# Sewer56/dxt-lossless-transform

Measured on AMD Instinct MI355X. Metric: GiB/s BC blocks transformed (fwd+inv), higher is better.
Workload: dtype u8

## Files before the change

### dxt-lossless-transform_amd/csrc/batch_api.cpp

```cpp
#include <hip/hip_runtime_api.h>

#include <algorithm>
#include <condition_variable>
#include <cstdlib>
#include <cstring>
#include <exception>
#include <mutex>
#include <thread>
#include <vector>

#include "../../include/dxtlt_gfx950.h"
#include "bcn_launch.h"
#include "granule_launch.h"
#include "host_common.h"
#include "table_ring.h"

namespace {

using namespace dxtlt_host;
using dxtlt::BatchEntry;

inline uint32_t item_block_bytes(uint8_t format)
{
    return is_pixel_format(format) ? (uint32_t)pixel_bytes_of(format) : format == 1 || format == 4 ? 8u : 16u;
}

const char* const kDeviceFormatText = "batch item: format must be 1..5 (BC1..BC5), 6 (BC6H) or 7 (BC7; 6 and 7 are this build's own formats; "
                                      "pixel formats 8 and 9 go through dxtlt_transform_batch_host or the calls of dxtlt_pixels.h)";
const char* const kHostFormatText = "batch item: format must be 1..5 (BC1..BC5), 6 (BC6H), 7 (BC7), 8 (4-byte pixels) or 9 (3-byte pixels; "
                                    "6 to 9 are this build's own formats)";

inline bool pixel_item_overlaps(const DxtltBatchItem& it)
{
    if (!is_pixel_format(it.format) || it.len == 0)
        return false;
    const uintptr_t a = reinterpret_cast<uintptr_t>(it.d_input), b = reinterpret_cast<uintptr_t>(it.d_output);
    return a < b + it.len && b < a + it.len;
}

int32_t launch_pixel_item(const DxtltBatchItem& it, void* stream)
{
    const uint64_t pixels = it.len / item_block_bytes(it.format);
    return pixel_device_range(pixel_bytes_of(it.format), it.inverse != 0, it.d_input, it.d_output, pixels, 0, pixels,
                              pixel_decorrelate_of(it.decorrelation_mode),
                              pixel_layout_of(it.split_alpha_endpoints != 0, it.split_colour_endpoints != 0), stream);
}

thread_local dxtlt_host::TableRing g_ring;

const bool kTableByCopyEngine = dxtlt::experiment_env("DXTLT_BATCH_TABLE_COPY") != nullptr && dxtlt::experiment_env("DXTLT_BATCH_TABLE_COPY")[0] == '1';

}

dxtlt_host::TableRing& dxtlt_host::thread_table_ring() { return g_ring; }

hipError_t dxtlt_host::upload_table(TableSlot* slot, size_t bytes, hipStream_t stream)
{
    if (kTableByCopyEngine)
        return hipMemcpyAsync(slot->dev, slot->host, bytes, hipMemcpyHostToDevice, stream);
    return dxtlt::launch_table_upload(slot->host_mapped, slot->dev, bytes, stream);
}

namespace {

int32_t batch_device(const DxtltBatchItem* items, size_t count, void* hip_stream, bool pixels_allowed)
{
    if (count == 0)
        return kOk;
    if (items == nullptr)
        return fail(kInvalidArgument, "NULL item array with count > 0");
    for (size_t i = 0; i < count; ++i) {
        const DxtltBatchItem& it = items[i];
        if (it.format < 1 || it.format > (pixels_allowed ? 9 : 7))
            return fail(kInvalidArgument, kDeviceFormatText);
        if (it.len % item_block_bytes(it.format) != 0)
            return fail(kInvalidLength, "batch item: len is not a multiple of the block size");
        if (it.decorrelation_mode > 3 && dxtlt::format_has_colour(it.format))
            return fail(kInvalidArgument, "batch item: decorrelation_mode must be 0..3");
        if (it.len > 0 && (it.d_input == nullptr || it.d_output == nullptr))
            return fail(kInvalidArgument, "batch item: NULL device buffer with len > 0");
        if (pixel_item_overlaps(it))
            return fail(kInvalidArgument, "batch item: pixel input and output overlap");
    }
    for (const int format : {7, 6}) {
        uint64_t granules[2] = {0, 0};
        for (size_t i = 0; i < count; ++i)
            if (items[i].format == format)
                granules[items[i].inverse ? 1 : 0] += items[i].len / 16 / 1024;
        if (granules[0] > 0xFFFFFFull || granules[1] > 0xFFFFFFull)
            return fail(kInvalidArgument, dxtlt::granule::named(format, "batch too large for one launch (256 GiB or more of ", " in one direction)"));
    }
    hipStream_t user = static_cast<hipStream_t>(hip_stream);

    struct Group {
        std::vector<BatchEntry> entries;
        uint32_t wgs = 0;
        uint32_t uniform_wgs = 0;
        bool uniform = true;
    };
    constexpr int kGroups = 5 * 2 * 16;
    std::vector<Group> groups(kGroups);
    auto group_settings = [](int gi) {
        dxtlt::Settings s{};
        s.variant = (gi >> 2) & 3;
        s.split_alpha = ((gi >> 1) & 1) != 0;
        s.split_colour = (gi & 1) != 0;
        return s;
    };
    std::vector<size_t> singles;
    for (size_t i = 0; i < count; ++i) {
        const DxtltBatchItem& it = items[i];
        if (it.len == 0 || dxtlt::granule::is_granule_format(it.format) || is_pixel_format(it.format))
            continue;
        if (it.len >= (size_t(64) << 30))
            return fail(kInvalidArgument, "batch item of 64 GiB or more: use the single-buffer entry point");
        const bool colour = dxtlt::format_has_colour(it.format);
        const int sa = dxtlt::format_has_alpha_split(it.format) && it.split_alpha_endpoints ? 1 : 0;
        const int sc = colour && it.split_colour_endpoints ? 1 : 0, mode = colour ? it.decorrelation_mode : 0;
        const int gi = (((it.format - 1) * 2 + (it.inverse ? 1 : 0)) << 4) | (mode << 2) | (sa << 1) | sc;
        Group& g = groups[gi];
        BatchEntry e{};
        e.src = static_cast<const uint8_t*>(it.d_input);
        e.dst = static_cast<uint8_t*>(it.d_output);
        e.blocks = it.len / item_block_bytes(it.format);
        e.first_wg = g.wgs;
        const uint32_t wgs = dxtlt::plan_batch_entry((dxtlt::Format)it.format, it.inverse != 0, group_settings(gi), e);
        if (wgs == 0xFFFFFFFFu) {
            singles.push_back(i);
            continue;
        }
        if ((uint64_t)g.wgs + wgs > 0xFFFFFFull)
            return fail(kInvalidArgument, "batch too large for one launch (64 GiB or more of one format, direction and settings)");
        g.wgs += wgs;
        g.entries.push_back(e);
        if (g.entries.size() == 1)
            g.uniform_wgs = wgs;
        else if (wgs != g.uniform_wgs)
            g.uniform = false;
    }
    static const bool no_uniform = dxtlt::experiment_env("DXTLT_BATCH_NO_UNIFORM") != nullptr;
    static const bool no_strided = dxtlt::experiment_env("DXTLT_BATCH_NO_STRIDED") != nullptr;

    using GranuleEntry = dxtlt::granule::BatchEntry;
    struct GranulePlan {
        std::vector<GranuleEntry> entries, tails;
        std::vector<uint32_t> coarse;
        uint64_t wgs = 0;
        size_t at = 0, entry_bytes = 0, tail_bytes = 0, bytes = 0;
    };
    GranulePlan granule_plans[4];
    size_t table_bytes = 0;
    for (int q = 0; q < 4; ++q) {
        GranulePlan& p = granule_plans[q];
        const int inverse = q & 1, format = q < 2 ? 7 : 6;
        for (size_t i = 0; i < count; ++i) {
            const DxtltBatchItem& it = items[i];
            if (it.format != format || it.len == 0 || (it.inverse != 0) != (inverse != 0))
                continue;
            const uint64_t blocks = it.len / 16, tail = blocks % 1024, main = blocks - tail;
            const uint8_t* src = static_cast<const uint8_t*>(it.d_input);
            uint8_t* dst = static_cast<uint8_t*>(it.d_output);
            if (main != 0) {
                p.entries.push_back({src, dst, main, (uint32_t)p.wgs, 0});
                p.wgs += main / 1024;
            }
            if (tail != 0)
                p.tails.push_back({src + main * 16, dst + main * 16, 0, 0, (uint32_t)tail});
        }
        if (p.entries.empty() && p.tails.empty())
            continue;
        p.coarse.resize(((size_t)p.wgs + 63) / 64);
        size_t cur = 0;
        for (size_t k = 0; k < p.coarse.size(); ++k) {
            while (cur + 1 < p.entries.size() && p.entries[cur + 1].first_wg <= (uint32_t)(k * 64))
                ++cur;
            p.coarse[k] = (uint32_t)cur;
        }
        p.entry_bytes = p.entries.size() * sizeof(GranuleEntry);
        p.tail_bytes = p.tails.size() * sizeof(GranuleEntry);
        p.bytes = (p.entry_bytes + p.tail_bytes + p.coarse.size() * sizeof(uint32_t) + 15) & ~(size_t)15;
        p.at = table_bytes;
        table_bytes += p.bytes;
    }

    struct Placed {
        int gi;
        size_t at, entry_bytes;
    };
    std::vector<Placed> placed;
    for (int gi = 0; gi < kGroups; ++gi) {
        const Group& g = groups[gi];
        if (g.entries.empty())
            continue;
        const size_t entry_bytes = (g.entries.size() * sizeof(BatchEntry) + 15) & ~(size_t)15;
        placed.push_back({gi, table_bytes, entry_bytes});
        table_bytes += entry_bytes + dxtlt::batch_index_bytes(g.wgs);
    }
    if (table_bytes != 0) {
        TableSlot* slot = nullptr;
        hipError_t e = g_ring.acquire(table_bytes, &slot);
        if (e != hipSuccess)
            return fail(kDevice, "batch table staging", e);
        for (const GranulePlan& p : granule_plans) {
            if (p.bytes == 0)
                continue;
            uint8_t* h = static_cast<uint8_t*>(slot->host) + p.at;
            if (p.entry_bytes) std::memcpy(h, p.entries.data(), p.entry_bytes);
            if (p.tail_bytes) std::memcpy(h + p.entry_bytes, p.tails.data(), p.tail_bytes);
            if (!p.coarse.empty()) std::memcpy(h + p.entry_bytes + p.tail_bytes, p.coarse.data(), p.coarse.size() * sizeof(uint32_t));
        }
        std::vector<bool> wide(placed.size());
        for (size_t k = 0; k < placed.size(); ++k) {
            const Group& g = groups[placed[k].gi];
            uint8_t* h = static_cast<uint8_t*>(slot->host) + placed[k].at;
            std::memcpy(h, g.entries.data(), g.entries.size() * sizeof(BatchEntry));
            wide[k] = dxtlt::build_batch_index(g.entries.data(), g.entries.size(), g.wgs, h + placed[k].entry_bytes);
        }
        e = upload_table(slot, table_bytes, user);
        const char* what = "batch table copy / launch";
        for (int q = 0; q < 4 && e == hipSuccess; ++q) {
            const GranulePlan& p = granule_plans[q];
            const int inverse = q & 1, format = q < 2 ? 7 : 6;
            if (p.bytes == 0)
                continue;
            const uint8_t* d = static_cast<const uint8_t*>(slot->dev) + p.at;
            e = dxtlt::granule::launch_batch(format, inverse != 0, reinterpret_cast<const GranuleEntry*>(d),
                                             reinterpret_cast<const uint32_t*>(d + p.entry_bytes + p.tail_bytes), (uint32_t)p.entries.size(),
                                             (uint32_t)p.wgs, reinterpret_cast<const GranuleEntry*>(d + p.entry_bytes),
                                             (uint32_t)p.tails.size(), user);
            if (e != hipSuccess)
                what = format == 7 ? "BC7 batch table copy / launch" : "BC6H batch table copy / launch";
        }
        for (size_t k = 0; k < placed.size() && e == hipSuccess; ++k) {
            const int gi = placed[k].gi;
            Group& g = groups[gi];
            const size_t n = g.entries.size();
            const bool uniform = g.uniform && !no_uniform;
            bool strided = uniform && !no_strided;
            const int64_t src_stride = n >= 2 ? (int64_t)(g.entries[1].src - g.entries[0].src) : 0;
            const int64_t dst_stride = n >= 2 ? (int64_t)(g.entries[1].dst - g.entries[0].dst) : 0;
            for (size_t i = 1; i < n && strided; ++i) {
                const BatchEntry &a = g.entries[0], &b = g.entries[i];
                strided = b.blocks == a.blocks && b.full_tiles == a.full_tiles && b.form == a.form && b.halo_vecs == a.halo_vecs &&
                          std::memcmp(b.shift, a.shift, sizeof a.shift) == 0 && std::memcmp(b.gbase, a.gbase, sizeof a.gbase) == 0 &&
                          b.src == a.src + (int64_t)i * src_stride && b.dst == a.dst + (int64_t)i * dst_stride;
            }
            const uint8_t* d = static_cast<const uint8_t*>(slot->dev) + placed[k].at;
            e = dxtlt::launch_batch((dxtlt::Format)((gi >> 5) + 1), ((gi >> 4) & 1) != 0, group_settings(gi),
                                    reinterpret_cast<const BatchEntry*>(d), d + placed[k].entry_bytes, (uint32_t)n, g.wgs,
                                    uniform ? g.uniform_wgs : 0, wide[k], user, strided ? &g.entries[0] : nullptr, src_stride, dst_stride);
        }
        hipError_t ev = hipEventRecord(slot->done, user);
        slot->pending = ev == hipSuccess;
        if (e != hipSuccess)
            return fail(kDevice, what, e);
        if (ev != hipSuccess)
            return fail(kDevice, "batch event", ev);
    }
    for (size_t i : singles) {
        const DxtltBatchItem& it = items[i];
        dxtlt::Settings s{};
        s.variant = it.decorrelation_mode;
        s.split_alpha = it.split_alpha_endpoints != 0;
        s.split_colour = it.split_colour_endpoints != 0;
        s = dxtlt::effective_settings((dxtlt::Format)it.format, s);
        const uint64_t blocks = it.len / item_block_bytes(it.format);
        const hipError_t e = dxtlt::launch_transform((dxtlt::Format)it.format, it.inverse != 0, s, it.d_input, it.d_output,
                                                     dxtlt::Range{blocks, 0, blocks}, user);
        if (e != hipSuccess)
            return fail(kDevice, "batch item launch", e);
    }
    for (size_t i = 0; i < count; ++i)
        if (is_pixel_format(items[i].format) && items[i].len != 0)
            if (int32_t rc = launch_pixel_item(items[i], user); rc != kOk)
                return rc;
    return kOk;
}

}

extern "C" int32_t dxtlt_transform_batch_device(const DxtltBatchItem* items, size_t count, void* hip_stream)
{
    return batch_device(items, count, hip_stream, false);
}

extern "C" uint32_t dxtlt_debug_plan_batch(int32_t format, int32_t inverse, int32_t variant, int32_t split_alpha, int32_t split_colour,
                                           const uint64_t* src_addresses, const uint64_t* dst_addresses, const uint64_t* blocks, size_t count,
                                           DxtltDebugPlannedEntry* entries_out, uint8_t* index_out, size_t index_capacity,
                                           uint32_t* index_is_wide_out)
{
    if (index_is_wide_out)
        *index_is_wide_out = 0;
    if (format < 1 || format > 5 || (count != 0 && (!src_addresses || !dst_addresses || !blocks || !entries_out)))
        return 0xFFFFFFFFu;
    dxtlt::Settings s{};
    s.variant = variant;
    s.split_alpha = split_alpha != 0;
    s.split_colour = split_colour != 0;
    s = dxtlt::effective_settings((dxtlt::Format)format, s);
    std::vector<BatchEntry> entries;
    uint32_t total = 0;
    for (size_t i = 0; i < count; ++i) {
        BatchEntry e{};
        e.src = reinterpret_cast<const uint8_t*>(static_cast<uintptr_t>(src_addresses[i]));
        e.dst = reinterpret_cast<uint8_t*>(static_cast<uintptr_t>(dst_addresses[i]));
        e.blocks = blocks[i];
        e.first_wg = total;
        const uint32_t wgs = dxtlt::plan_batch_entry((dxtlt::Format)format, inverse != 0, s, e);
        if (wgs == 0xFFFFFFFFu || (uint64_t)total + wgs > 0xFFFFFFull)
            return 0xFFFFFFFFu;
        if (wgs == 0)
            e.end_wg = e.first_wg;
        total += wgs;
        DxtltDebugPlannedEntry& o = entries_out[i];
        o.first_wg = e.first_wg;
        o.end_wg = e.end_wg;
        o.full_tiles = e.full_tiles;
        o.form = e.form;
        o.halo_vecs = e.halo_vecs;
        std::memcpy(o.shift, e.shift, sizeof o.shift);
        std::memcpy(o.gbase, e.gbase, sizeof o.gbase);
        if (wgs != 0)
            entries.push_back(e);
    }
    if (total != 0) {
        if (index_out == nullptr || index_capacity < dxtlt::batch_index_bytes(total))
            return 0xFFFFFFFFu;
        const bool wide = dxtlt::build_batch_index(entries.data(), entries.size(), total, index_out);
        if (index_is_wide_out)
            *index_is_wide_out = wide ? 1 : 0;
    }
    return total;
}

namespace {

size_t env_number(const char* name, size_t fallback)
{
    const char* v = std::getenv(name);
    const unsigned long long x = v ? std::strtoull(v, nullptr, 10) : 0;
    return x ? (size_t)x : fallback;
}
const size_t kHostBatchChunkBytes = env_number("DXTLT_BATCH_CHUNK_MIB", 64) << 20;
const int kCopyThreads = (int)std::min<size_t>(64, env_number("DXTLT_BATCH_THREADS", 6));

struct PinnedArenas {
    void* in[2] = {nullptr, nullptr};
    void* out[2] = {nullptr, nullptr};
    size_t cap = 0;
    ~PinnedArenas() { release(); }
    void release()
    {
        for (int i = 0; i < 2; ++i) {
            if (in[i]) (void)hipHostFree(in[i]);
            if (out[i]) (void)hipHostFree(out[i]);
            in[i] = out[i] = nullptr;
        }
        cap = 0;
    }
    hipError_t reserve(size_t bytes)
    {
        if (bytes <= cap)
            return hipSuccess;
        release();
        for (int i = 0; i < 2; ++i) {
            hipError_t e = hipHostMalloc(&in[i], bytes, hipHostMallocDefault);
            if (e == hipSuccess)
                e = hipHostMalloc(&out[i], bytes, hipHostMallocDefault);
            if (e != hipSuccess) {
                release();
                return e;
            }
        }
        cap = bytes;
        return hipSuccess;
    }
};
thread_local PinnedArenas g_pinned;
#define g_pinned_in(c) (pinned_in[(c) & 1])
#define g_pinned_out(c) (pinned_out[(c) & 1])

struct HostBatchShared {
    std::mutex m;
    std::condition_variable cv;
    std::vector<int> packed;
    std::vector<int> unpacked;
    int uploaded_recorded = 0;
    int kernels_issued = 0;
    int enqueued = 0;
    bool failed = false;
    hipError_t error = hipSuccess;
};

}

void dxtlt_host::release_batch_thread_tables()
{
    g_ring.release();
    g_pinned.release();
}

extern "C" int32_t dxtlt_transform_batch_host(const DxtltBatchItem* items, size_t count)
{
    if (count == 0)
        return kOk;
    if (items == nullptr)
        return fail(kInvalidArgument, "NULL item array with count > 0");
    uint64_t total = 0;
    for (size_t i = 0; i < count; ++i) {
        const DxtltBatchItem& it = items[i];
        if (it.format < 1 || it.format > 9)
            return fail(kInvalidArgument, kHostFormatText);
        if (it.len % item_block_bytes(it.format) != 0)
            return fail(kInvalidLength, "batch item: len is not a multiple of the block size");
        if (it.decorrelation_mode > 3 && dxtlt::format_has_colour(it.format))
            return fail(kInvalidArgument, "batch item: decorrelation_mode must be 0..3");
        if (it.len > 0 && (it.d_input == nullptr || it.d_output == nullptr))
            return fail(kInvalidArgument, "batch item: NULL buffer with len > 0");
        if (pixel_item_overlaps(it))
            return fail(kInvalidArgument, "batch item: pixel input and output overlap");
        if (it.len >= (size_t(4) << 30))
            return fail(kInvalidArgument, "batch item of 4 GiB or more: use the single-buffer entry point");
        total += (it.len + 255) & ~uint64_t(255);
    }
    if (total == 0)
        return kOk;

    const uint64_t big_item = 2 * (uint64_t)kHostBatchChunkBytes;
    std::vector<DxtltBatchItem> small;
    small.reserve(count);
    for (size_t i = 0; i < count; ++i) {
        const DxtltBatchItem& it = items[i];
        if (it.len < big_item) {
            small.push_back(it);
            continue;
        }
        int32_t rc;
        if (is_pixel_format(it.format))
            rc = pixel_host_call(pixel_bytes_of(it.format), it.inverse != 0, static_cast<const uint8_t*>(it.d_input),
                                 static_cast<uint8_t*>(it.d_output), it.len, pixel_decorrelate_of(it.decorrelation_mode),
                                 pixel_layout_of(it.split_alpha_endpoints != 0, it.split_colour_endpoints != 0));
        else if (dxtlt::granule::is_granule_format(it.format))
            rc = dxtlt_host::granule_host_call(it.format, it.inverse != 0, static_cast<const uint8_t*>(it.d_input),
                                               static_cast<uint8_t*>(it.d_output), it.len);
        else
            rc = dxtlt_host::transform(it.format, it.inverse != 0, static_cast<const uint8_t*>(it.d_input),
                                       static_cast<uint8_t*>(it.d_output), it.len, it.decorrelation_mode,
                                       dxtlt::format_has_alpha_split(it.format) && it.split_alpha_endpoints, it.split_colour_endpoints != 0);
        if (rc != kOk)
            return rc;
    }
    if (small.empty())
        return kOk;
    items = small.data();
    count = small.size();

    std::vector<uint64_t> slot(count);
    std::vector<size_t> chunk_first;
    std::vector<uint64_t> chunk_bytes;
    {
        uint64_t in_chunk = 0;
        chunk_first.push_back(0);
        for (size_t i = 0; i < count; ++i) {
            const uint64_t padded = (items[i].len + 255) & ~uint64_t(255);
            if (in_chunk > 0 && in_chunk + padded > kHostBatchChunkBytes) {
                chunk_first.push_back(i);
                chunk_bytes.push_back(in_chunk);
                in_chunk = 0;
            }
            slot[i] = in_chunk;
            in_chunk += padded;
        }
        chunk_first.push_back(count);
        chunk_bytes.push_back(in_chunk);
    }
    const int nchunks = (int)chunk_bytes.size();
    const uint64_t arena_bytes = *std::max_element(chunk_bytes.begin(), chunk_bytes.end());

    void *d_in = nullptr, *d_out = nullptr;
    hipStream_t up = nullptr;
    if (int32_t rc = acquire_staging((size_t)(2 * arena_bytes), &d_in, &d_out, &up); rc != kOk)
        return rc;
    if (hipError_t e = g_pinned.reserve((size_t)arena_bytes); e != hipSuccess)
        return fail(kDevice, "hipHostMalloc(batch arenas)", e);
    void* const pinned_in[2] = {g_pinned.in[0], g_pinned.in[1]};
    void* const pinned_out[2] = {g_pinned.out[0], g_pinned.out[1]};
    int dev = 0;
    (void)hipGetDevice(&dev);
    hipStream_t down = nullptr;
    if (hipError_t e = hipStreamCreateWithFlags(&down, hipStreamNonBlocking); e != hipSuccess)
        return fail(kDevice, "hipStreamCreate(download)", e);

    std::vector<hipEvent_t> ev((size_t)nchunks * 3, nullptr);
    for (auto& e : ev)
        if (hipError_t err = hipEventCreateWithFlags(&e, hipEventDisableTiming); err != hipSuccess) {
            for (auto& e2 : ev) if (e2) (void)hipEventDestroy(e2);
            (void)hipStreamDestroy(down);
            return fail(kDevice, "hipEventCreate", err);
        }
    auto ev_uploaded = [&](int c) { return ev[(size_t)c * 3]; };
    auto ev_kernels = [&](int c) { return ev[(size_t)c * 3 + 1]; };
    auto ev_downloaded = [&](int c) { return ev[(size_t)c * 3 + 2]; };

    HostBatchShared sh;
    sh.packed.assign((size_t)nchunks, 0);
    sh.unpacked.assign((size_t)nchunks, 0);
    auto set_failed = [&](hipError_t e) {
        std::lock_guard<std::mutex> lk(sh.m);
        if (!sh.failed) {
            sh.failed = true;
            sh.error = e;
        }
        sh.cv.notify_all();
    };

    auto packer = [&](int tid) {
        hipError_t e = hipSetDevice(dev);
        for (int c = 0; c < nchunks && e == hipSuccess; ++c) {
            if (c < 2) {
                std::lock_guard<std::mutex> lk(sh.m);
                if (sh.failed)
                    return;
            }
            if (c >= 2) {
                {
                    std::unique_lock<std::mutex> lk(sh.m);
                    sh.cv.wait(lk, [&] { return sh.uploaded_recorded > c - 2 || sh.failed; });
                    if (sh.failed)
                        return;
                }
                e = hipEventSynchronize(ev_uploaded(c - 2));
                if (e != hipSuccess)
                    break;
            }
            uint8_t* arena = static_cast<uint8_t*>(g_pinned_in(c));
            for (size_t i = chunk_first[(size_t)c] + (size_t)tid; i < chunk_first[(size_t)c + 1]; i += kCopyThreads)
                if (items[i].len)
                    std::memcpy(arena + slot[i], items[i].d_input, items[i].len);
            {
                std::lock_guard<std::mutex> lk(sh.m);
                sh.packed[(size_t)c]++;
            }
            sh.cv.notify_all();
        }
        if (e != hipSuccess)
            set_failed(e);
    };
    auto unpacker = [&](int tid) {
        hipError_t e = hipSetDevice(dev);
        for (int c = 0; c < nchunks && e == hipSuccess; ++c) {
            {
                std::unique_lock<std::mutex> lk(sh.m);
                sh.cv.wait(lk, [&] { return sh.enqueued > c || sh.failed; });
                if (sh.enqueued <= c)
                    return;
            }
            e = hipEventSynchronize(ev_downloaded(c));
            if (e != hipSuccess)
                break;
            const uint8_t* arena = static_cast<const uint8_t*>(g_pinned_out(c));
            for (size_t i = chunk_first[(size_t)c] + (size_t)tid; i < chunk_first[(size_t)c + 1]; i += kCopyThreads)
                if (items[i].len)
                    std::memcpy(items[i].d_output, arena + slot[i], items[i].len);
            {
                std::lock_guard<std::mutex> lk(sh.m);
                sh.unpacked[(size_t)c]++;
            }
            sh.cv.notify_all();
        }
        if (e != hipSuccess)
            set_failed(e);
    };

    std::vector<std::thread> threads;
    bool spawn_failed = false;
    auto spawn = [&](auto&& fn, auto... args) {
        if (spawn_failed)
            return;
        try {
            threads.emplace_back(fn, args...);
        } catch (const std::exception&) {
            spawn_failed = true;
        }
    };
    for (int t = 0; t < kCopyThreads; ++t) spawn(packer, t);
    for (int t = 0; t < kCopyThreads; ++t) spawn(unpacker, t);

    auto downloader = [&] {
        hipError_t e = hipSetDevice(dev);
        for (int c = 0; c < nchunks && e == hipSuccess; ++c) {
            {
                std::unique_lock<std::mutex> lk(sh.m);
                sh.cv.wait(lk, [&] { return (sh.kernels_issued > c && (c < 2 || sh.unpacked[(size_t)c - 2] == kCopyThreads)) || sh.failed; });
                if (sh.failed)
                    return;
            }
            const uint8_t* dout = static_cast<const uint8_t*>(d_out) + (size_t)(c & 1) * arena_bytes;
            e = hipStreamWaitEvent(down, ev_kernels(c), 0);
            if (e == hipSuccess)
                e = hipMemcpyAsync(g_pinned_out(c), dout, (size_t)chunk_bytes[(size_t)c], hipMemcpyDeviceToHost, down);
            if (e == hipSuccess)
                e = hipEventRecord(ev_downloaded(c), down);
            if (e != hipSuccess)
                break;
            {
                std::lock_guard<std::mutex> lk(sh.m);
                sh.enqueued = c + 1;
            }
            sh.cv.notify_all();
        }
        if (e != hipSuccess)
            set_failed(e);
    };
    spawn(downloader);
    if (spawn_failed) {
        set_failed(hipErrorOutOfMemory);
        for (auto& t : threads)
            t.join();
        for (auto& e : ev) (void)hipEventDestroy(e);
        (void)hipStreamDestroy(down);
        return fail(kAllocation, "could not start the batch copy threads");
    }

    int32_t rc = kOk;
    hipError_t err = hipSuccess;
    std::vector<DxtltBatchItem> dev_items;
    for (int c = 0; c < nchunks && rc == kOk && err == hipSuccess; ++c) {
        {
            std::unique_lock<std::mutex> lk(sh.m);
            sh.cv.wait(lk, [&] { return (sh.packed[(size_t)c] == kCopyThreads && (c < 2 || sh.enqueued > c - 2)) || sh.failed; });
            if (sh.failed)
                break;
        }
        uint8_t* di = static_cast<uint8_t*>(d_in) + (size_t)(c & 1) * arena_bytes;
        uint8_t* dout = static_cast<uint8_t*>(d_out) + (size_t)(c & 1) * arena_bytes;
        if (c >= 2)
            err = hipStreamWaitEvent(up, ev_kernels(c - 2), 0);
        if (err == hipSuccess)
            err = hipMemcpyAsync(di, g_pinned_in(c), (size_t)chunk_bytes[(size_t)c], hipMemcpyHostToDevice, up);
        if (err == hipSuccess)
            err = hipEventRecord(ev_uploaded(c), up);
        {
            std::lock_guard<std::mutex> lk(sh.m);
            if (err == hipSuccess)
                sh.uploaded_recorded = c + 1;
        }
        sh.cv.notify_all();
        if (err != hipSuccess)
            break;
        if (c >= 2)
            err = hipStreamWaitEvent(up, ev_downloaded(c - 2), 0);
        if (err != hipSuccess)
            break;
        dev_items.clear();
        for (size_t i = chunk_first[(size_t)c]; i < chunk_first[(size_t)c + 1]; ++i) {
            DxtltBatchItem it = items[i];
            it.d_input = di + slot[i];
            it.d_output = dout + slot[i];
            dev_items.push_back(it);
        }
        rc = batch_device(dev_items.data(), dev_items.size(), up, true);
        if (rc != kOk)
            break;
        err = hipEventRecord(ev_kernels(c), up);
        if (err != hipSuccess)
            break;
        {
            std::lock_guard<std::mutex> lk(sh.m);
            sh.kernels_issued = c + 1;
        }
        sh.cv.notify_all();
    }
    if (rc != kOk || err != hipSuccess) {
        std::lock_guard<std::mutex> lk(sh.m);
        sh.failed = true;
        if (err != hipSuccess && sh.error == hipSuccess)
            sh.error = err;
        sh.cv.notify_all();
    }
    for (auto& t : threads)
        t.join();
    (void)hipStreamSynchronize(up);
    (void)hipStreamSynchronize(down);
    for (auto& e : ev) (void)hipEventDestroy(e);
    (void)hipStreamDestroy(down);
    if (rc != kOk)
        return rc;
    if (sh.failed)
        return fail(kDevice, "host batch copy", sh.error);
    return kOk;
}
```

### dxt-lossless-transform_amd/csrc/batch_kernels.hip

```cpp
#include <cstdlib>
#include <cstring>
#include <vector>

#include "bcn_device.h"

#include "batch_lookup.h"

namespace dxtlt {

struct BatchView {
    const uint8_t* src;
    uint8_t* dst;
    uint64_t blocks;
    uint32_t first_wg, end_wg, full_tiles;
    uint32_t flags;
    uint32_t shifts[2];
    uint64_t gbase[6];
};

__device__ __forceinline__ BatchView load_batch_entry(const BatchEntry* entry)
{
    const uint64_t* q = reinterpret_cast<const uint64_t*>(entry);
    const uint32_t* w = reinterpret_cast<const uint32_t*>(entry);
    BatchView v;
    v.src = (const uint8_t*)(global_cptr)q[0];
    v.dst = (uint8_t*)(global_ptr)q[1];
    v.blocks = q[2];
    v.first_wg = w[6];
    v.end_wg = w[7];
    v.full_tiles = w[8];
    v.flags = w[9];
    v.shifts[0] = w[10];
    v.shifts[1] = w[11];
#pragma unroll
    for (int i = 0; i < 6; ++i)
        v.gbase[i] = q[6 + i];
    return v;
}
__device__ __forceinline__ void pin_batch_view(BatchView& v)
{
#ifdef DXTLT_WG_TIMING
    (void)v;
    return;
#endif
    uint64_t s = reinterpret_cast<uintptr_t>(v.src), d = reinterpret_cast<uintptr_t>(v.dst);
    asm("" : "+s"(s), "+s"(d), "+s"(v.blocks));
    v.src = (const uint8_t*)(global_cptr)s;
    v.dst = (uint8_t*)(global_ptr)d;
    asm("" : "+s"(v.first_wg), "+s"(v.end_wg), "+s"(v.full_tiles), "+s"(v.flags), "+s"(v.shifts[0]), "+s"(v.shifts[1]));
#pragma unroll
    for (int i = 0; i < 6; ++i)
        asm("" : "+s"(v.gbase[i]));
}
static_assert(offsetof(BatchEntry, first_wg) == 24 && offsetof(BatchEntry, end_wg) == 28 && offsetof(BatchEntry, full_tiles) == 32 && offsetof(BatchEntry, form) == 36 &&
                  offsetof(BatchEntry, shift) == 40 && offsetof(BatchEntry, gbase) == 48,
              "load_batch_entry reads BatchEntry by dword offsets");

constexpr uint32_t kBatchAligned = 1;

struct StridedBatch {
    BatchEntry first;
    int64_t src_stride, dst_stride;
    uint32_t on;
};

#ifdef DXTLT_WG_TIMING
__device__ uint32_t g_wg_timing[4 << 20];
extern "C" int dxtlt_debug_read_wg_timing(uint32_t* out, size_t count)
{
    return (int)hipMemcpyFromSymbol(out, HIP_SYMBOL(g_wg_timing), count * 4);
}
extern "C" int dxtlt_debug_read_wg_marks(uint32_t* out, size_t count)
{
    return (int)hipMemcpyFromSymbol(out, HIP_SYMBOL(dxtlt::g_wg_marks), count * 4);
}
#define WG_TIMING_BEGIN const uint64_t t_begin = __builtin_amdgcn_s_memrealtime();
#define WG_TIMING_END(kind)                                                                         \
    do {                                                                                            \
        __builtin_amdgcn_s_waitcnt(0);                                                              \
        asm volatile("s_waitcnt vmcnt(0)" ::: "memory");                                            \
        if (threadIdx.x == 0 && blockIdx.x < (1u << 20)) {                                          \
            uint32_t xcc;                                                                           \
            asm volatile("s_getreg_b32 %0, hwreg(HW_REG_XCC_ID)" : "=s"(xcc));                       \
            g_wg_timing[4 * blockIdx.x] = (uint32_t)(__builtin_amdgcn_s_memrealtime() - t_begin);   \
            g_wg_timing[4 * blockIdx.x + 1] = (kind);                                               \
            g_wg_timing[4 * blockIdx.x + 2] = (uint32_t)t_begin;                                    \
            g_wg_timing[4 * blockIdx.x + 3] = xcc & 0xF;                                            \
        }                                                                                           \
    } while (0)
#else
#define WG_TIMING_BEGIN
#define WG_TIMING_END(kind)
#endif

template <int FMT, int VARIANT, bool SA, bool SC, bool INVERSE, int THREADS = batch_tile_threads(FMT, SC, INVERSE)>
__global__ void __launch_bounds__(THREADS)
batch_kernel(const BatchEntry* __restrict__ entries_arg, const uint8_t* __restrict__ index_arg, uint32_t n_base, uint32_t uniform_wgs,
             uint32_t magic, StridedBatch strided)
{
    constexpr int kLds = INVERSE ? shift_lds_bytes(1, THREADS) : halo_lds_bytes<FMT, THREADS>();
    __shared__ __attribute__((aligned(16))) uint8_t lds[kLds];
    const uint32_t wg = blockIdx.x;
    WG_TIMING_BEGIN
    BatchView en;
    uint32_t e;
    uint64_t entries_at = reinterpret_cast<uintptr_t>(entries_arg), index_at = reinterpret_cast<uintptr_t>(index_arg);
#ifndef DXTLT_WG_TIMING
    asm("" : "+s"(entries_at), "+s"(index_at), "+s"(n_base), "+s"(uniform_wgs), "+s"(magic));
#endif
    const BatchEntry* entries = (const BatchEntry*)(const __attribute__((address_space(1))) BatchEntry*)entries_at;
    const uint8_t* index = (const uint8_t*)(global_cptr)index_at;
    if (uniform_wgs != 0) {
        e = __umulhi(wg, magic);
        if ((e + 1) * uniform_wgs <= wg)
            ++e;
        if (strided.on != 0) {
            const BatchEntry& f = strided.first;
            en.src = (const uint8_t*)(global_cptr)(reinterpret_cast<uintptr_t>(f.src) + (uint64_t)((int64_t)e * strided.src_stride));
            en.dst = (uint8_t*)(global_ptr)(reinterpret_cast<uintptr_t>(f.dst) + (uint64_t)((int64_t)e * strided.dst_stride));
            en.blocks = f.blocks;
            en.first_wg = e * uniform_wgs;
            en.end_wg = en.first_wg + uniform_wgs;
            en.full_tiles = f.full_tiles;
            en.flags = (uint32_t)f.form | ((uint32_t)f.halo_vecs << 8) | ((uint32_t)f.natural << 16);
            en.shifts[0] = (uint32_t)f.shift[0] | ((uint32_t)f.shift[1] << 8) | ((uint32_t)f.shift[2] << 16) | ((uint32_t)f.shift[3] << 24);
            en.shifts[1] = (uint32_t)f.shift[4] | ((uint32_t)f.shift[5] << 8);
#pragma unroll
            for (int i = 0; i < 6; ++i)
                en.gbase[i] = f.gbase[i];
        } else {
            en = load_batch_entry(entries + e);
        }
    } else {
        e = batch_entry_of_workgroup(entries, index, n_base, magic, wg, en);
    }
    const uint32_t n_wgs = en.end_wg - en.first_wg;
    uint32_t local = wg - en.first_wg;
    if (n_wgs >= 8) {
        local += (en.first_wg + n_wgs - 1u - e) & 7u;
        local = local >= n_wgs ? local - n_wgs : local;
    }
    const bool aligned = (en.flags & 0xFF) == kBatchAligned;
    if (aligned && local < en.full_tiles) {
        if constexpr (INVERSE)
            inv_aligned_tile<FMT, VARIANT, SA, SC, THREADS>(en.src, en.dst, en.blocks, 0, local, lds);
        else
            fwd_aligned_tile<FMT, VARIANT, SA, SC, THREADS>(en.src, en.dst, en.blocks, 0, local, lds);
        WG_TIMING_END(1);
        return;
    }
    Shifts sh;
#pragma unroll
    for (int i = 0; i < 6; ++i) {
        sh.d[i] = (int)((en.shifts[i >> 2] >> (8 * (i & 3))) & 127u);
        sh.gbase[i] = en.gbase[i];
    }
#ifdef DXTLT_EXPERIMENTS
    sh.xcd_remap = 0;
    sh.line_policy = INVERSE ? 1 : 3;
    sh.skip_partial = 0;
#endif
    sh.natural = 1;
    sh.halo_vecs = (int)(en.flags >> 8) & 0xFF;
    sh.full_tiles = en.full_tiles;
    sh.range_blocks = en.blocks;
    if constexpr (INVERSE) {
        if (local < en.full_tiles) {
            const uint64_t tile = xcd_contiguous_tile(local, en.full_tiles);
            inv_shift_tile<FMT, VARIANT, SA, SC, THREADS>(en.src, en.dst, en.blocks, 0, sh, tile, lds);
            WG_TIMING_END(2);
            return;
        }
        inv_shift_edge_tile<FMT, VARIANT, SA, SC, THREADS>(en.src, en.dst, en.blocks, sh, en.full_tiles, lds);
        WG_TIMING_END(4);
    } else {
        if (local != 0 && local < en.full_tiles) {
            fwd_halo_tile<FMT, VARIANT, SA, SC, kNormNone, true, THREADS>(en.src, en.dst, en.blocks, 0, sh, local, lds);
            WG_TIMING_END(2);
            return;
        }
        fwd_halo_edge_tile<FMT, VARIANT, SA, SC, kNormNone, true, THREADS>(en.src, en.dst, sh, local, lds);
        WG_TIMING_END(local == 0 ? 3 : 4);
    }
}

uint32_t plan_batch_entry(Format fmt, bool inverse, const Settings& s, BatchEntry& e)
{
    if (e.blocks == 0)
        return 0;
    const Settings es = effective_settings(fmt, s);
    const Streams S = make_streams(fmt, es.split_alpha, es.split_colour);
    const void* soa = inverse ? (const void*)e.src : (const void*)e.dst;
    const uint64_t T = (uint64_t)tile_blocks(fmt, batch_tile_threads(fmt, es.split_colour, inverse));
    const uint64_t tiles = e.blocks / T, rest = e.blocks % T;
    const uint64_t mask = inverse ? 15 : (uint64_t)(kHaloAlign - 1);
    bool on_lines = true, stream_tails = false;
    int d[6] = {0, 0, 0, 0, 0, 0}, halo_blocks = 0;
    for (int i = 0; i < S.n; ++i) {
        const uint64_t base = reinterpret_cast<uintptr_t>(soa) + (uint64_t)S.off[i] * e.blocks;
        d[i] = (int)(base & mask);
        on_lines = on_lines && (base & 127) == 0;
        stream_tails = stream_tails || d[i] != 0;
        halo_blocks = std::max(halo_blocks, (d[i] + S.width[i] - 1) / S.width[i]);
    }
    if (!shifts_are_natural(S, d))
        return 0xFFFFFFFFu;
    e.form = on_lines ? 1 : 0;
    e.natural = 1;
    e.reserved = 0;
    e.reserved2[0] = e.reserved2[1] = 0;
    const int per_vec = 16 / fmt_block(fmt);
    e.halo_vecs = inverse ? 0 : (uint8_t)((halo_blocks + per_vec - 1) / per_vec);
    for (int i = 0; i < 6; ++i) {
        e.shift[i] = (uint8_t)d[i];
        e.gbase[i] = i < S.n ? (uint64_t)S.off[i] * e.blocks - (uint64_t)d[i] : 0;
    }
    e.full_tiles = (uint32_t)tiles;
    const bool edge = rest != 0 || (!inverse && stream_tails);
    const uint32_t wgs = (uint32_t)tiles + (edge ? 1u : 0u);
    e.end_wg = e.first_wg + wgs;
    return wgs;
}

bool build_batch_index(const BatchEntry* entries, size_t n_entries, uint32_t total_wgs, uint8_t* index)
{
    const size_t n_base = batch_index_base_count(total_wgs), n_delta = batch_index_delta_count(total_wgs);
    uint32_t* base = reinterpret_cast<uint32_t*>(index);
    std::memset(index, 0, batch_index_bytes(total_wgs));
    std::vector<uint32_t> d(n_delta);
    uint32_t largest = 0;
    size_t cur = 0;
    for (size_t j = 0; j < n_delta; ++j) {
        const uint32_t wg = (uint32_t)(j * kBatchIndexWgs);
        while (cur + 1 < n_entries && entries[cur].end_wg <= wg)
            ++cur;
        if (wg % kBatchBaseWgs == 0)
            base[wg / kBatchBaseWgs] = (uint32_t)cur;
        d[j] = (uint32_t)(cur - base[wg / kBatchBaseWgs]);
        largest = std::max(largest, d[j]);
    }
    const bool wide = largest > 255;
    uint8_t* delta = index + n_base * 4;
    for (size_t j = 0; j < n_delta; ++j) {
        if (wide) {
            delta[2 * j] = (uint8_t)d[j];
            delta[2 * j + 1] = (uint8_t)(d[j] >> 8);
        } else {
            delta[j] = (uint8_t)d[j];
        }
    }
    return wide;
}

namespace {

using BatchFn = void (*)(const BatchEntry*, const uint8_t*, uint32_t, uint32_t, uint32_t, StridedBatch);

template <int FMT, int VARIANT, bool SA, bool SC>
BatchFn batch_fn(bool inverse) { return inverse ? batch_kernel<FMT, VARIANT, SA, SC, true> : batch_kernel<FMT, VARIANT, SA, SC, false>; }

template <int FMT, int VARIANT>
BatchFn batch_splits(bool sa, bool sc, bool inverse)
{
    if constexpr (FMT == kBc3) {
        if (sa)
            return sc ? batch_fn<FMT, VARIANT, true, true>(inverse) : batch_fn<FMT, VARIANT, true, false>(inverse);
    }
    return sc ? batch_fn<FMT, VARIANT, false, true>(inverse) : batch_fn<FMT, VARIANT, false, false>(inverse);
}

template <int FMT>
BatchFn batch_bc45(bool split_endpoints, bool inverse)
{
    return split_endpoints ? batch_fn<FMT, kNone, true, false>(inverse) : batch_fn<FMT, kNone, false, false>(inverse);
}

template <int FMT>
BatchFn batch_variant(int variant, bool sa, bool sc, bool inverse)
{
    switch (variant) {
    case kNone: return batch_splits<FMT, kNone>(sa, sc, inverse);
    case kVar1: return batch_splits<FMT, kVar1>(sa, sc, inverse);
    case kVar2: return batch_splits<FMT, kVar2>(sa, sc, inverse);
    default: return batch_splits<FMT, kVar3>(sa, sc, inverse);
    }
}

}

hipError_t launch_batch(Format fmt, bool inverse, const Settings& s, const BatchEntry* d_entries, const uint8_t* d_index,
                        uint32_t n_entries, uint32_t total_wgs, uint32_t uniform_wgs, bool wide_index, hipStream_t stream,
                        const BatchEntry* strided_first, int64_t src_stride, int64_t dst_stride)
{
    if (n_entries == 0 || total_wgs == 0)
        return hipSuccess;
    if (s.variant < 0 || s.variant > 3 || total_wgs > 0xFFFFFFu)
        return hipErrorInvalidValue;
    if (uniform_wgs != 0 && (uint64_t)uniform_wgs * n_entries != total_wgs)
        return hipErrorInvalidValue;
    const uint32_t magic = uniform_wgs > 1 ? (uint32_t)((1ull << 32) / uniform_wgs) : uniform_wgs == 1 ? 0xFFFFFFFFu : n_entries;
    static const bool no_array = experiment_env("DXTLT_BATCH_NO_ARRAY") != nullptr;
    if (strided_first != nullptr && uniform_wgs != 0 && !no_array && strided_first->form == 1) {
        const hipError_t e = launch_tiled_array(fmt, inverse, s, strided_first->src, strided_first->dst, strided_first->blocks, n_entries,
                                                src_stride, dst_stride, stream);
        if (e != hipErrorNotSupported)
            return e;
    }
    StridedBatch strided{};
    if (strided_first != nullptr && uniform_wgs != 0) {
        strided.first = *strided_first;
        strided.src_stride = src_stride;
        strided.dst_stride = dst_stride;
        strided.on = 1;
    }
    const Settings es = effective_settings(fmt, s);
    const bool sa = es.split_alpha, sc = es.split_colour;
    BatchFn k = nullptr;
    switch (fmt) {
    case kBc1: k = batch_variant<kBc1>(es.variant, false, sc, inverse); break;
    case kBc2: k = batch_variant<kBc2>(es.variant, false, sc, inverse); break;
    case kBc3: k = batch_variant<kBc3>(es.variant, sa, sc, inverse); break;
    case kBc4: k = batch_bc45<kBc4>(sa, inverse); break;
    case kBc5: k = batch_bc45<kBc5>(sa, inverse); break;
    default: return hipErrorInvalidValue;
    }
    hipLaunchKernelGGL(k, dim3(total_wgs), dim3(batch_tile_threads(fmt, sc, inverse)), 0, stream, d_entries, d_index,
                       (uint32_t)batch_index_base_count(total_wgs) | (wide_index ? 0x80000000u : 0u), uniform_wgs, magic, strided);
    return hipGetLastError();
}

}
```

### dxt-lossless-transform_amd/csrc/batch_lookup.h

```cpp
#pragma once
#include <stddef.h>
#include <stdint.h>

namespace dxtlt {

template <typename ENTRY, typename VIEW>
__device__ __forceinline__ uint32_t batch_entry_of_workgroup(const ENTRY* entries, const uint8_t* index, uint32_t n_base,
                                                             uint32_t n_entries, uint32_t wg, VIEW& en)
{
    static_assert(offsetof(ENTRY, end_wg) == 28, "the bisection reads end_wg as dword 7 of an entry");
    const uint32_t* base = reinterpret_cast<const uint32_t*>(index);
    const uint32_t wide = n_base >> 31;
    const uint8_t* delta = index + (n_base & 0x7FFFFFFFu) * 4;
    uint32_t e = base[wg >> 12];
    const uint32_t dword = reinterpret_cast<const uint32_t*>(delta)[wg >> (8u - wide)];
    e += (dword >> (((wg >> 6) & (3u >> wide)) << (3u + wide))) & (0xFFu | (wide * 0xFF00u));
    en = load_batch_entry(entries + e);
    pin_batch_view(en);
    if (en.end_wg <= wg) {
        uint32_t lo = e + 1, hi = e + (wg & 63u);
        hi = hi < n_entries - 1u ? hi : n_entries - 1u;
        while (lo < hi) {
            const uint32_t mid = (lo + hi) >> 1;
            const uint32_t end = reinterpret_cast<const uint32_t*>(entries + mid)[7];
            lo = end <= wg ? mid + 1 : lo;
            hi = end <= wg ? hi : mid;
        }
        e = lo;
        en = load_batch_entry(entries + e);
    }
    return e;
}

__device__ __forceinline__ uint32_t batch_rotated_tile(uint32_t first_wg, uint32_t end_wg, uint32_t e, uint32_t wg)
{
    const uint32_t n_wgs = end_wg - first_wg;
    uint32_t local = wg - first_wg;
    if (n_wgs >= 8) {
        local += (first_wg + n_wgs - 1u - e) & 7u;
        local = local >= n_wgs ? local - n_wgs : local;
    }
    return local;
}

}
```

### dxt-lossless-transform_amd/csrc/bcn_device.h

```cpp
#pragma once
#include <hip/hip_runtime.h>

#include <algorithm>
#include <cstddef>
#include <type_traits>

#include "bc1_normalize.h"
#include "bcn_launch.h"
#include "streaming_store.h"
#include "ycocg_swar.h"

namespace dxtlt {

typedef uint32_t u32x4 __attribute__((ext_vector_type(4)));
typedef uint32_t u32x2 __attribute__((ext_vector_type(2)));

constexpr int kThreads = 256;
constexpr int default_tile_threads(int fmt, bool inverse)
{
    (void)inverse;
    return fmt == kBc1 || fmt == kBc4 ? 128 : 256;
}

#ifndef DXTLT_NONTEMPORAL
#define DXTLT_NONTEMPORAL 1
#endif

#ifdef DXTLT_WG_TIMING
__device__ uint32_t g_wg_marks[8 << 20];
__device__ __forceinline__ void wg_mark(int i)
{
    if (threadIdx.x == 0 && blockIdx.x < (1u << 20))
        g_wg_marks[8 * blockIdx.x + i] = (uint32_t)__builtin_amdgcn_s_memrealtime();
}
#define WG_MARK(i) wg_mark(i)
#define WG_MARK_LOADS_DONE(i)                                  \
    do {                                                       \
        asm volatile("s_waitcnt vmcnt(0)" ::: "memory");       \
        wg_mark(i);                                            \
    } while (0)
#else
#define WG_MARK(i)
#define WG_MARK_LOADS_DONE(i)
#endif

__device__ __forceinline__ u32x4 gload16(const void* p)
{
#if DXTLT_NONTEMPORAL
    return __builtin_nontemporal_load(reinterpret_cast<const u32x4*>(p));
#else
    return *reinterpret_cast<const u32x4*>(p);
#endif
}

__device__ __forceinline__ void gstore16(void* p, u32x4 v)
{
#if DXTLT_NONTEMPORAL
    store_streaming16(p, v);
#else
    *reinterpret_cast<u32x4*>(p) = v;
#endif
}

__device__ __forceinline__ void gstore16_aos(uint8_t* aos_base, void* p, u32x4 v)
{
    if ((reinterpret_cast<uintptr_t>(aos_base) & 15) == 0)
        gstore16(p, v);
    else
        __builtin_nontemporal_store(v, reinterpret_cast<u32x4*>(p));
}

template <int I, int N, typename F>
__device__ __forceinline__ void static_for(F&& f)
{
    if constexpr (I < N) {
        f(std::integral_constant<int, I>{});
        static_for<I + 1, N>(f);
    }
}

template <int W, int WAVES, typename F>
__device__ __forceinline__ void for_this_wave_from(int w, F&& f)
{
    if constexpr (W + 1 >= WAVES) {
        f(std::integral_constant<int, W>{});
    } else {
        if (w == W)
            f(std::integral_constant<int, W>{});
        else
            for_this_wave_from<W + 1, WAVES>(w, f);
    }
}
template <int WAVES, typename F>
__device__ __forceinline__ void for_this_wave(int t, F&& f)
{
    for_this_wave_from<0, WAVES>(__builtin_amdgcn_readfirstlane(t >> 6), f);
}

__host__ __device__ constexpr int fmt_block(int fmt) { return fmt == kBc1 || fmt == kBc4 ? 8 : 16; }
__host__ __device__ constexpr int tile_blocks(int fmt, int threads) { return threads * 16 / fmt_block(fmt); }

template <int FMT, bool SA, bool SC, int T>
__device__ __forceinline__ uint64_t soa_offset_of_image_byte(int o, uint64_t total_blocks, uint64_t blk0)
{
    constexpr Streams S = make_streams(FMT, SA, SC);
    uint64_t r = 0;
#pragma unroll
    for (int s = 0; s < S.n; ++s) {
        const int lo = S.off[s] * T;
        const int hi = lo + S.width[s] * T;
        if (o >= lo && o < hi)
            r = (uint64_t)S.off[s] * total_blocks + (uint64_t)S.width[s] * blk0 + (uint64_t)(o - lo);
    }
    return r;
}

#ifndef DXTLT_WAVE_OFFSETS
#define DXTLT_WAVE_OFFSETS 1
#endif
template <int FMT, bool SA, bool SC, int T, int W>
__device__ __forceinline__ uint64_t soa_offset_of_image_byte_in_wave(int o, uint64_t total_blocks, uint64_t blk0)
{
    constexpr Streams S = make_streams(FMT, SA, SC);
    constexpr int wave_lo = W * 1024, wave_hi = wave_lo + 1024;
    uint64_t r = 0;
    static_for<0, S.n>([&](auto si) {
        constexpr int s = decltype(si)::value;
        constexpr int lo = S.off[s] * T;
        constexpr int hi = lo + S.width[s] * T;
        if constexpr (lo < wave_hi && hi > wave_lo) {
            constexpr bool only = lo <= wave_lo && hi >= wave_hi;
            const uint64_t base = (uint64_t)S.off[s] * total_blocks + (uint64_t)S.width[s] * blk0;
            if (only || (o >= lo && o < hi))
                r = base + (uint64_t)(uint32_t)(o - lo);
        }
    });
    return r;
}

template <int FMT, bool SA, bool SC, int THREADS>
__device__ __forceinline__ uint64_t soa_offset_of_lane(int t, uint64_t total_blocks, uint64_t blk0)
{
    constexpr int T = tile_blocks(FMT, THREADS);
#if DXTLT_WAVE_OFFSETS
    uint64_t o = 0;
    for_this_wave<THREADS / 64>(t, [&](auto wi) {
        o = soa_offset_of_image_byte_in_wave<FMT, SA, SC, T, decltype(wi)::value>(t * 16, total_blocks, blk0);
    });
    return o;
#else
    return soa_offset_of_image_byte<FMT, SA, SC, T>(t * 16, total_blocks, blk0);
#endif
}

template <typename T>
__device__ __forceinline__ T& lds_at(uint8_t* lds, int byte_off)
{
    return *reinterpret_cast<T*>(lds + byte_off);
}

typedef volatile uint16_t __attribute__((address_space(3))) lds_halfword;
__device__ __forceinline__ lds_halfword* lds_halfwords(uint8_t* lds, int byte_off)
{
    return (lds_halfword*)(lds + byte_off);
}

#ifndef DXTLT_BC3_RECORD6
#define DXTLT_BC3_RECORD6 1
#endif
typedef uint32_t u32x2_align4 __attribute__((ext_vector_type(2), aligned(4)));
typedef volatile uint32_t __attribute__((address_space(3))) lds_dword;

__device__ __forceinline__ void lds_put_record6(uint8_t* lds, int addr, uint32_t lo16, uint32_t hi32)
{
#if DXTLT_BC3_RECORD6
    const bool odd = (addr & 2) != 0;
    const int a32 = odd ? addr + 2 : addr;
    const int a16 = odd ? addr : addr + 4;
    const uint32_t v32 = odd ? hi32 : (lo16 & 0xFFFFu) | (hi32 << 16);
    const uint32_t v16 = odd ? lo16 : hi32 >> 16;
    *(lds_dword*)(lds + a32) = v32;
    *lds_halfwords(lds, a16) = (uint16_t)v16;
#else
    lds_halfwords(lds, addr)[0] = (uint16_t)lo16;
    lds_halfwords(lds, addr)[1] = (uint16_t)hi32;
    lds_halfwords(lds, addr)[2] = (uint16_t)(hi32 >> 16);
#endif
}

__device__ __forceinline__ void lds_get_record6(uint8_t* lds, int addr, uint32_t& lo16, uint32_t& hi32)
{
#if DXTLT_BC3_RECORD6
    const u32x2_align4 w = *reinterpret_cast<const u32x2_align4*>(lds + (addr & ~3));
    const uint32_t sh = (uint32_t)(addr & 2) * 8u;
    const uint32_t rec = __builtin_amdgcn_alignbit(w.y, w.x, sh);
    lo16 = rec & 0xFFFFu;
    hi32 = (rec >> 16) | ((w.y >> sh) << 16);
#else
    lo16 = lds_at<uint16_t>(lds, addr + 0);
    hi32 = (uint32_t)lds_at<uint16_t>(lds, addr + 2) | ((uint32_t)lds_at<uint16_t>(lds, addr + 4) << 16);
#endif
}

template <bool SA, int T, int E>
__device__ __forceinline__ void scatter_bc4_half(uint8_t* lds, int b, uint32_t lo, uint32_t hi)
{
    if constexpr (SA) {
        lds_at<uint8_t>(lds, E * T + b) = (uint8_t)lo;
        lds_at<uint8_t>(lds, (E + 1) * T + b) = (uint8_t)(lo >> 8);
    } else {
        lds_at<uint16_t>(lds, E * T + 2 * b) = (uint16_t)lo;
    }
    lds_put_record6(lds, (E + 2) * T + 6 * b, lo >> 16, hi);
}

template <bool SA, int T, int E>
__device__ __forceinline__ void gather_bc4_half(uint8_t* lds, int b, uint32_t& lo, uint32_t& hi)
{
    uint32_t a01;
    if constexpr (SA)
        a01 = (uint32_t)lds_at<uint8_t>(lds, E * T + b) | ((uint32_t)lds_at<uint8_t>(lds, (E + 1) * T + b) << 8);
    else
        a01 = lds_at<uint16_t>(lds, E * T + 2 * b);
    uint32_t i01;
    lds_get_record6(lds, (E + 2) * T + 6 * b, i01, hi);
    lo = a01 | (i01 << 16);
}

template <int FMT, int VARIANT, bool SA, bool SC, int T>
__device__ __forceinline__ void scatter_to_image(uint8_t* lds, int u, u32x4 q)
{
    if constexpr (FMT == kBc4) {
        if constexpr (SA) {
            lds_at<uint16_t>(lds, 0 * T + 2 * u) = (uint16_t)((q.x & 0xFFu) | ((q.z & 0xFFu) << 8));
            lds_at<uint16_t>(lds, 1 * T + 2 * u) = (uint16_t)(((q.x >> 8) & 0xFFu) | (q.z & 0xFF00u));
        } else {
            lds_at<uint32_t>(lds, 0 * T + 4 * u) = (q.x & 0xFFFFu) | (q.z << 16);
        }
        lds_at<uint32_t>(lds, 2 * T + 12 * u + 0) = (q.x >> 16) | (q.y << 16);
        lds_at<uint32_t>(lds, 2 * T + 12 * u + 4) = (q.y >> 16) | (q.z & 0xFFFF0000u);
        lds_at<uint32_t>(lds, 2 * T + 12 * u + 8) = q.w;
    } else if constexpr (FMT == kBc5) {
        scatter_bc4_half<SA, T, 0>(lds, u, q.x, q.y);
        scatter_bc4_half<SA, T, 8>(lds, u, q.z, q.w);
    } else if constexpr (FMT == kBc1) {
        const uint32_t ca = decorrelate2<VARIANT>(q.x);
        const uint32_t cb = decorrelate2<VARIANT>(q.z);
        if constexpr (SC) {
            lds_at<uint32_t>(lds, 0 * T + 4 * u) = (ca & 0xFFFFu) | (cb << 16);
            lds_at<uint32_t>(lds, 2 * T + 4 * u) = (ca >> 16) | (cb & 0xFFFF0000u);
        } else {
            lds_at<u32x2>(lds, 0 * T + 8 * u) = u32x2{ca, cb};
        }
        lds_at<u32x2>(lds, 4 * T + 8 * u) = u32x2{q.y, q.w};
    } else if constexpr (FMT == kBc2) {
        const uint32_t c = decorrelate2<VARIANT>(q.z);
        lds_at<u32x2>(lds, 0 * T + 8 * u) = u32x2{q.x, q.y};
        if constexpr (SC) {
            lds_at<uint16_t>(lds, 8 * T + 2 * u) = (uint16_t)c;
            lds_at<uint16_t>(lds, 10 * T + 2 * u) = (uint16_t)(c >> 16);
        } else {
            lds_at<uint32_t>(lds, 8 * T + 4 * u) = c;
        }
        lds_at<uint32_t>(lds, 12 * T + 4 * u) = q.w;
    } else {
        const uint32_t c = decorrelate2<VARIANT>(q.z);
        if constexpr (SA) {
            lds_at<uint8_t>(lds, 0 * T + u) = (uint8_t)q.x;
            lds_at<uint8_t>(lds, 1 * T + u) = (uint8_t)(q.x >> 8);
        } else {
            lds_at<uint16_t>(lds, 0 * T + 2 * u) = (uint16_t)q.x;
        }
        lds_put_record6(lds, 2 * T + 6 * u, q.x >> 16, q.y);
        if constexpr (SC) {
            lds_at<uint16_t>(lds, 8 * T + 2 * u) = (uint16_t)c;
            lds_at<uint16_t>(lds, 10 * T + 2 * u) = (uint16_t)(c >> 16);
        } else {
            lds_at<uint32_t>(lds, 8 * T + 4 * u) = c;
        }
        lds_at<uint32_t>(lds, 12 * T + 4 * u) = q.w;
    }
}

template <int FMT, int VARIANT, bool SA, bool SC, int T>
__device__ __forceinline__ u32x4 gather_from_image(uint8_t* lds, int u)
{
    u32x4 q;
    if constexpr (FMT == kBc4) {
        uint32_t e;
        if constexpr (SA) {
            const uint32_t a0 = lds_at<uint16_t>(lds, 0 * T + 2 * u), a1 = lds_at<uint16_t>(lds, 1 * T + 2 * u);
            e = (a0 & 0xFFu) | ((a1 & 0xFFu) << 8) | ((a0 & 0xFF00u) << 8) | ((a1 & 0xFF00u) << 16);
        } else {
            e = lds_at<uint32_t>(lds, 0 * T + 4 * u);
        }
        const uint32_t r0 = lds_at<uint32_t>(lds, 2 * T + 12 * u + 0);
        const uint32_t r1 = lds_at<uint32_t>(lds, 2 * T + 12 * u + 4);
        const uint32_t r2 = lds_at<uint32_t>(lds, 2 * T + 12 * u + 8);
        q.x = (e & 0xFFFFu) | (r0 << 16);
        q.y = (r0 >> 16) | (r1 << 16);
        q.z = (e >> 16) | (r1 & 0xFFFF0000u);
        q.w = r2;
    } else if constexpr (FMT == kBc5) {
        uint32_t rlo, rhi, glo, ghi;
        gather_bc4_half<SA, T, 0>(lds, u, rlo, rhi);
        gather_bc4_half<SA, T, 8>(lds, u, glo, ghi);
        q = u32x4{rlo, rhi, glo, ghi};
    } else if constexpr (FMT == kBc1) {
        uint32_t ca, cb;
        if constexpr (SC) {
            const uint32_t c0 = lds_at<uint32_t>(lds, 0 * T + 4 * u);
            const uint32_t c1 = lds_at<uint32_t>(lds, 2 * T + 4 * u);
            ca = (c0 & 0xFFFFu) | (c1 << 16);
            cb = (c0 >> 16) | (c1 & 0xFFFF0000u);
        } else {
            const u32x2 p = lds_at<u32x2>(lds, 0 * T + 8 * u);
            ca = p.x;
            cb = p.y;
        }
        const u32x2 idx = lds_at<u32x2>(lds, 4 * T + 8 * u);
        q.x = recorrelate2<VARIANT>(ca);
        q.y = idx.x;
        q.z = recorrelate2<VARIANT>(cb);
        q.w = idx.y;
    } else if constexpr (FMT == kBc2) {
        const u32x2 a = lds_at<u32x2>(lds, 0 * T + 8 * u);
        uint32_t c;
        if constexpr (SC)
            c = (uint32_t)lds_at<uint16_t>(lds, 8 * T + 2 * u) | ((uint32_t)lds_at<uint16_t>(lds, 10 * T + 2 * u) << 16);
        else
            c = lds_at<uint32_t>(lds, 8 * T + 4 * u);
        q.x = a.x;
        q.y = a.y;
        q.z = recorrelate2<VARIANT>(c);
        q.w = lds_at<uint32_t>(lds, 12 * T + 4 * u);
    } else {
        uint32_t a01;
        if constexpr (SA)
            a01 = (uint32_t)lds_at<uint8_t>(lds, 0 * T + u) | ((uint32_t)lds_at<uint8_t>(lds, 1 * T + u) << 8);
        else
            a01 = lds_at<uint16_t>(lds, 0 * T + 2 * u);
        uint32_t i01, i2345;
        lds_get_record6(lds, 2 * T + 6 * u, i01, i2345);
        uint32_t c;
        if constexpr (SC)
            c = (uint32_t)lds_at<uint16_t>(lds, 8 * T + 2 * u) | ((uint32_t)lds_at<uint16_t>(lds, 10 * T + 2 * u) << 16);
        else
            c = lds_at<uint32_t>(lds, 8 * T + 4 * u);
        q.x = a01 | (i01 << 16);
        q.y = i2345;
        q.z = recorrelate2<VARIANT>(c);
        q.w = lds_at<uint32_t>(lds, 12 * T + 4 * u);
    }
    return q;
}

__device__ __forceinline__ uint64_t xcd_contiguous_tile(uint32_t orig, uint32_t nwg)
{
    const uint32_t q = nwg >> 3, r = nwg & 7, xcd = orig & 7;
    const uint32_t start = xcd < r ? xcd * (q + 1) : r * (q + 1) + (xcd - r) * q;
    return start + (orig >> 3);
}


template <int FMT, int NORM>
__device__ __forceinline__ u32x4 normalize_vector(u32x4 q)
{
    if constexpr (FMT == kBc1 && NORM != kNormNone) {
        uint32_t ca = q.x, xa = q.y, cb = q.z, xb = q.w;
        normalize_bc1_block<NORM>(ca, xa);
        normalize_bc1_block<NORM>(cb, xb);
        q = u32x4{ca, xa, cb, xb};
    }
    return q;
}

constexpr int kTiledArray = 2;

template <int FMT, int VARIANT, bool SA, bool SC, int THREADS, int NORM = kNormNone>
__device__ __forceinline__ void fwd_aligned_tile(const uint8_t* __restrict__ aos, uint8_t* __restrict__ soa,
                                                 uint64_t total_blocks, uint64_t first_block, uint64_t tile, uint8_t* lds)
{
    constexpr int T = tile_blocks(FMT, THREADS);
    const int t = threadIdx.x;
    WG_MARK(1);
    const u32x4 q = normalize_vector<FMT, NORM>(gload16(aos + tile * (THREADS * 16) + t * 16));
    WG_MARK_LOADS_DONE(2);
    scatter_to_image<FMT, VARIANT, SA, SC, T>(lds, t, q);
    __syncthreads();
    WG_MARK(3);
    const u32x4 v = lds_at<u32x4>(lds, t * 16);
    const uint64_t o = soa_offset_of_lane<FMT, SA, SC, THREADS>(t, total_blocks, first_block + tile * T);
    gstore16(soa + o, v);
    WG_MARK(4);
}

struct AosSink {
    template <int FMT, int THREADS>
    __device__ __forceinline__ void store(uint8_t* aos, uint64_t tile, int t, u32x4 q) const
    {
        gstore16_aos(aos, aos + tile * (THREADS * 16) + t * 16, q);
    }
    template <int FMT, int THREADS>
    __device__ __forceinline__ void store_edge(uint8_t* aos, uint64_t tile, int t, u32x4 q, int own) const
    {
        constexpr int PV = 16 / fmt_block(FMT);
        uint8_t* out = aos + tile * (THREADS * 16) + t * 16;
        if ((t + 1) * PV <= own)
            __builtin_nontemporal_store(q, reinterpret_cast<u32x4*>(out));
        else
            __builtin_nontemporal_store(u32x2{q.x, q.y}, reinterpret_cast<u32x2*>(out));
    }
};

template <int FMT, int VARIANT, bool SA, bool SC, int THREADS, typename SINK = AosSink>
__device__ __forceinline__ void inv_aligned_tile(const uint8_t* __restrict__ soa, uint8_t* __restrict__ aos,
                                                 uint64_t total_blocks, uint64_t first_block, uint64_t tile, uint8_t* lds,
                                                 const SINK& sink = SINK{})
{
    constexpr int T = tile_blocks(FMT, THREADS);
    const int t = threadIdx.x;
    const uint64_t o = soa_offset_of_lane<FMT, SA, SC, THREADS>(t, total_blocks, first_block + tile * T);
    lds_at<u32x4>(lds, t * 16) = gload16(soa + o);
    __syncthreads();
    const u32x4 q = gather_from_image<FMT, VARIANT, SA, SC, T>(lds, t);
    sink.template store<FMT, THREADS>(aos, tile, t, q);
}

template <int FMT, int VARIANT, bool SA, bool SC, int THREADS, int NORM = kNormNone>
__global__ void __launch_bounds__(THREADS)
fwd_tiled(const uint8_t* __restrict__ aos, uint8_t* __restrict__ soa, uint64_t total_blocks, uint64_t first_block,
          int xcd_remap, int64_t aos_stride, int64_t soa_stride)
{
    __shared__ __attribute__((aligned(16))) uint8_t lds[THREADS * 16];
    WG_MARK(0);
    if (xcd_remap & kTiledArray) {
        aos += (int64_t)blockIdx.y * aos_stride;
        soa += (int64_t)blockIdx.y * soa_stride;
    }
#ifdef DXTLT_EXPERIMENTS
    const uint64_t tile = (xcd_remap & 1) ? xcd_contiguous_tile(blockIdx.x, gridDim.x) : (uint64_t)blockIdx.x;
#else
    const uint64_t tile = blockIdx.x;
#endif
    fwd_aligned_tile<FMT, VARIANT, SA, SC, THREADS, NORM>(aos, soa, total_blocks, first_block, tile, lds);
}

template <int FMT, int VARIANT, bool SA, bool SC, int THREADS>
__global__ void __launch_bounds__(THREADS)
inv_tiled(const uint8_t* __restrict__ soa, uint8_t* __restrict__ aos, uint64_t total_blocks, uint64_t first_block,
          int xcd_remap, int64_t soa_stride, int64_t aos_stride)
{
    __shared__ __attribute__((aligned(16))) uint8_t lds[THREADS * 16];
    if (xcd_remap & kTiledArray) {
        soa += (int64_t)blockIdx.y * soa_stride;
        aos += (int64_t)blockIdx.y * aos_stride;
    }
#ifdef DXTLT_EXPERIMENTS
    const uint64_t tile = (xcd_remap & 1) ? xcd_contiguous_tile(blockIdx.x, gridDim.x) : (uint64_t)blockIdx.x;
#else
    const uint64_t tile = blockIdx.x;
#endif
    inv_aligned_tile<FMT, VARIANT, SA, SC, THREADS>(soa, aos, total_blocks, first_block, tile, lds);
}

struct Shifts {
    int d[6];
    int natural;
    int halo_vecs;
    uint64_t gbase[6];
    uint32_t full_tiles;
    uint64_t range_blocks;
#ifdef DXTLT_EXPERIMENTS
    int xcd_remap;
    int line_policy;
    int skip_partial;
#endif
};

__device__ __forceinline__ bool shifts_xcd_contiguous(const Shifts& sh, bool product_default)
{
#ifdef DXTLT_EXPERIMENTS
    (void)product_default;
    return sh.xcd_remap != 0;
#else
    (void)sh;
    return product_default;
#endif
}
__device__ __forceinline__ bool shifts_halo_write_through(const Shifts& sh)
{
#ifdef DXTLT_EXPERIMENTS
    return sh.line_policy == 3;
#else
    (void)sh;
    return true;
#endif
}
__device__ __forceinline__ bool shifts_skip_partial(const Shifts& sh)
{
#ifdef DXTLT_EXPERIMENTS
    return sh.skip_partial != 0;
#else
    (void)sh;
    return false;
#endif
}

template <typename STREAMS>
__host__ __device__ inline void fill_gbase(Shifts& sh, const STREAMS& S, uint64_t total_blocks, uint64_t first_block)
{
    for (int i = 0; i < 6; ++i)
        sh.gbase[i] = i < S.n ? (uint64_t)S.off[i] * total_blocks + (uint64_t)S.width[i] * first_block - (uint64_t)sh.d[i] : 0;
}

typedef const __attribute__((address_space(1))) uint8_t* global_cptr;
typedef __attribute__((address_space(1))) uint8_t* global_ptr;

__device__ __forceinline__ const uint8_t* fetched_now(const uint8_t* p)
{
    uint64_t v = reinterpret_cast<uintptr_t>(p);
    asm("" : "+s"(v));
    return (const uint8_t*)(global_cptr)v;
}
__device__ __forceinline__ uint8_t* fetched_now(uint8_t* p)
{
    uint64_t v = reinterpret_cast<uintptr_t>(p);
    asm("" : "+s"(v));
    return (uint8_t*)(global_ptr)v;
}

__device__ __forceinline__ Shifts shifts_fetched_at_once(const Shifts& in)
{
    Shifts s = in;
#ifdef DXTLT_EXPERIMENTS
    asm("" : "+s"(s.d[0]), "+s"(s.d[1]), "+s"(s.d[2]), "+s"(s.d[3]), "+s"(s.d[4]), "+s"(s.d[5]), "+s"(s.gbase[0]), "+s"(s.gbase[1]),
             "+s"(s.gbase[2]), "+s"(s.gbase[3]), "+s"(s.gbase[4]), "+s"(s.gbase[5]), "+s"(s.xcd_remap), "+s"(s.line_policy),
             "+s"(s.skip_partial), "+s"(s.natural), "+s"(s.halo_vecs), "+s"(s.full_tiles), "+s"(s.range_blocks));
#else
    asm("" : "+s"(s.d[0]), "+s"(s.d[1]), "+s"(s.d[2]), "+s"(s.d[3]), "+s"(s.d[4]), "+s"(s.d[5]), "+s"(s.gbase[0]), "+s"(s.gbase[1]),
             "+s"(s.gbase[2]), "+s"(s.gbase[3]), "+s"(s.gbase[4]), "+s"(s.gbase[5]), "+s"(s.natural), "+s"(s.halo_vecs),
             "+s"(s.full_tiles), "+s"(s.range_blocks));
#endif
    return s;
}

__host__ __device__ constexpr int stream_element_width(int bytes_per_block) { return bytes_per_block == 6 ? 2 : bytes_per_block; }

template <typename STREAMS>
__host__ __device__ inline int shifts_are_natural(const STREAMS& S, const int (&d)[6])
{
    int ok = 1;
    for (int i = 0; i < 6; ++i)
        if (i < S.n && (d[i] & (stream_element_width(S.width[i]) - 1)) != 0)
            ok = 0;
    return ok;
}


template <typename T>
using lds_volatile = volatile T __attribute__((address_space(3)));

template <int SIZE>
__device__ __forceinline__ void lds_put_piece(uint8_t* lds, int addr, uint64_t v)
{
    if constexpr (SIZE == 1) *(lds_volatile<uint8_t>*)(lds + addr) = (uint8_t)v;
    if constexpr (SIZE == 2) *(lds_volatile<uint16_t>*)(lds + addr) = (uint16_t)v;
    if constexpr (SIZE == 4) *(lds_volatile<uint32_t>*)(lds + addr) = (uint32_t)v;
    if constexpr (SIZE == 8) *(lds_volatile<uint64_t>*)(lds + addr) = v;
}

template <int SIZE>
__device__ __forceinline__ uint64_t lds_get_piece(uint8_t* lds, int addr)
{
    if constexpr (SIZE == 1) return *(lds_volatile<uint8_t>*)(lds + addr);
    if constexpr (SIZE == 2) return *(lds_volatile<uint16_t>*)(lds + addr);
    if constexpr (SIZE == 4) return *(lds_volatile<uint32_t>*)(lds + addr);
    if constexpr (SIZE == 8) return *(lds_volatile<uint64_t>*)(lds + addr);
    return 0;
}

constexpr int lds_piece_size(int W, int K, int P)
{
    const int a = K + P;
    int align = a == 0 ? W : (a & -a);
    if (align > W) align = W;
    int size = 1;
    while (size * 2 <= align && size * 2 <= W - P) size *= 2;
    return size;
}

template <int W, int K, int P = 0>
__device__ __forceinline__ void lds_put_seq(uint8_t* lds, int addr, uint64_t v)
{
    if constexpr (P < W) {
        constexpr int size = lds_piece_size(W, K, P);
        lds_put_piece<size>(lds, addr + P, v >> (8 * P));
        lds_put_seq<W, K, P + size>(lds, addr, v);
    }
}

template <int W, int K, int P = 0>
__device__ __forceinline__ uint64_t lds_get_seq(uint8_t* lds, int addr)
{
    if constexpr (P < W) {
        constexpr int size = lds_piece_size(W, K, P);
        return (lds_get_piece<size>(lds, addr + P) << (8 * P)) | lds_get_seq<W, K, P + size>(lds, addr);
    }
    return 0;
}

template <int W, bool NAT = false>
__device__ __forceinline__ void lds_put(uint8_t* lds, int addr, uint64_t v)
{
    if constexpr (W == 1 || NAT) {
        lds_put_piece<W>(lds, addr, v);
    } else {
        switch (addr & (W - 1)) {
        case 0: lds_put_seq<W, 0>(lds, addr, v); break;
        case 1: lds_put_seq<W, 1>(lds, addr, v); break;
        case 2: if constexpr (W > 2) lds_put_seq<W, 2>(lds, addr, v); break;
        case 3: if constexpr (W > 2) lds_put_seq<W, 3>(lds, addr, v); break;
        case 4: if constexpr (W > 4) lds_put_seq<W, 4>(lds, addr, v); break;
        case 5: if constexpr (W > 4) lds_put_seq<W, 5>(lds, addr, v); break;
        case 6: if constexpr (W > 4) lds_put_seq<W, 6>(lds, addr, v); break;
        default: if constexpr (W > 4) lds_put_seq<W, 7>(lds, addr, v); break;
        }
    }
}

template <int W, bool NAT = false>
__device__ __forceinline__ uint64_t lds_get(uint8_t* lds, int addr)
{
    if constexpr (W == 1 || NAT) {
        return lds_get_piece<W>(lds, addr);
    } else {
        switch (addr & (W - 1)) {
        case 0: return lds_get_seq<W, 0>(lds, addr);
        case 1: return lds_get_seq<W, 1>(lds, addr);
        case 2: if constexpr (W > 2) return lds_get_seq<W, 2>(lds, addr); break;
        case 3: if constexpr (W > 2) return lds_get_seq<W, 3>(lds, addr); break;
        case 4: if constexpr (W > 4) return lds_get_seq<W, 4>(lds, addr); break;
        case 5: if constexpr (W > 4) return lds_get_seq<W, 5>(lds, addr); break;
        case 6: if constexpr (W > 4) return lds_get_seq<W, 6>(lds, addr); break;
        default: if constexpr (W > 4) return lds_get_seq<W, 7>(lds, addr); break;
        }
        return 0;
    }
}

template <int FMT, bool SA, bool SC>
struct FieldStreams {
    static constexpr int alpha = 0;
    static constexpr int a1 = 1;
    static constexpr int aidx = SA ? 2 : 1;
    static constexpr int col = FMT == kBc1 ? 0 : FMT == kBc2 ? 1 : (SA ? 3 : 2);
    static constexpr int c1 = col + 1;
    static constexpr int idx = col + (SC ? 2 : 1);
    static constexpr int galpha = aidx + 1;
    static constexpr int ga1 = galpha + 1;
    static constexpr int gaidx = SA ? galpha + 2 : galpha + 1;
};

template <bool SA, bool NAT, int ALPHA, int A1, int AIDX>
__device__ __forceinline__ void scatter_shifted_bc4_block(uint8_t* lds, int b, uint32_t lo, uint32_t hi, const int (&base)[6])
{
    if constexpr (SA) {
        lds_put<1>(lds, base[ALPHA] + b, lo & 0xFF);
        lds_put<1>(lds, base[A1] + b, (lo >> 8) & 0xFF);
    } else {
        lds_put<2, NAT>(lds, base[ALPHA] + 2 * b, lo & 0xFFFF);
    }
    if constexpr (NAT && DXTLT_BC3_RECORD6) {
        lds_put_record6(lds, base[AIDX] + 6 * b, lo >> 16, hi);
    } else {
        lds_put<2, NAT>(lds, base[AIDX] + 6 * b + 0, lo >> 16);
        lds_put<2, NAT>(lds, base[AIDX] + 6 * b + 2, hi & 0xFFFF);
        lds_put<2, NAT>(lds, base[AIDX] + 6 * b + 4, hi >> 16);
    }
}

template <bool SA, bool NAT, int ALPHA, int A1, int AIDX>
__device__ __forceinline__ void gather_shifted_bc4_block(uint8_t* lds, int b, uint32_t& lo, uint32_t& hi, const int (&base)[6])
{
    uint32_t a01;
    if constexpr (SA)
        a01 = (uint32_t)lds_get<1>(lds, base[ALPHA] + b) | ((uint32_t)lds_get<1>(lds, base[A1] + b) << 8);
    else
        a01 = (uint32_t)lds_get<2, NAT>(lds, base[ALPHA] + 2 * b);
    if constexpr (NAT && DXTLT_BC3_RECORD6) {
        uint32_t i01;
        lds_get_record6(lds, base[AIDX] + 6 * b, i01, hi);
        lo = a01 | (i01 << 16);
    } else {
        const uint32_t i01 = (uint32_t)lds_get<2, NAT>(lds, base[AIDX] + 6 * b + 0);
        const uint32_t i23 = (uint32_t)lds_get<2, NAT>(lds, base[AIDX] + 6 * b + 2);
        const uint32_t i45 = (uint32_t)lds_get<2, NAT>(lds, base[AIDX] + 6 * b + 4);
        lo = a01 | (i01 << 16);
        hi = i23 | (i45 << 16);
    }
}

template <int FMT, int VARIANT, bool SA, bool SC, bool NAT>
__device__ __forceinline__ void scatter_shifted(uint8_t* lds, int u, u32x4 q, const int (&base)[6])
{
    using F = FieldStreams<FMT, SA, SC>;
    if constexpr (FMT == kBc4) {
        scatter_shifted_bc4_block<SA, NAT, F::alpha, F::a1, F::aidx>(lds, 2 * u, q.x, q.y, base);
        scatter_shifted_bc4_block<SA, NAT, F::alpha, F::a1, F::aidx>(lds, 2 * u + 1, q.z, q.w, base);
    } else if constexpr (FMT == kBc5) {
        scatter_shifted_bc4_block<SA, NAT, F::alpha, F::a1, F::aidx>(lds, u, q.x, q.y, base);
        scatter_shifted_bc4_block<SA, NAT, F::galpha, F::ga1, F::gaidx>(lds, u, q.z, q.w, base);
    } else if constexpr (FMT == kBc1) {
        const uint32_t ca = decorrelate2<VARIANT>(q.x);
        const uint32_t cb = decorrelate2<VARIANT>(q.z);
        if constexpr (NAT) {
            if constexpr (SC) {
                lds_put<2, true>(lds, base[F::col] + 4 * u, ca & 0xFFFFu);
                lds_put<2, true>(lds, base[F::col] + 4 * u + 2, cb & 0xFFFFu);
                lds_put<2, true>(lds, base[F::c1] + 4 * u, ca >> 16);
                lds_put<2, true>(lds, base[F::c1] + 4 * u + 2, cb >> 16);
            } else {
                lds_put<4, true>(lds, base[F::col] + 8 * u, ca);
                lds_put<4, true>(lds, base[F::col] + 8 * u + 4, cb);
            }
            lds_put<4, true>(lds, base[F::idx] + 8 * u, q.y);
            lds_put<4, true>(lds, base[F::idx] + 8 * u + 4, q.w);
        } else {
            if constexpr (SC) {
                lds_put<4>(lds, base[F::col] + 4 * u, (ca & 0xFFFFu) | (cb << 16));
                lds_put<4>(lds, base[F::c1] + 4 * u, (ca >> 16) | (cb & 0xFFFF0000u));
            } else {
                lds_put<8>(lds, base[F::col] + 8 * u, (uint64_t)ca | ((uint64_t)cb << 32));
            }
            lds_put<8>(lds, base[F::idx] + 8 * u, (uint64_t)q.y | ((uint64_t)q.w << 32));
        }
    } else {
        const uint32_t c = decorrelate2<VARIANT>(q.z);
        if constexpr (FMT == kBc2) {
            lds_put<8, NAT>(lds, base[F::alpha] + 8 * u, (uint64_t)q.x | ((uint64_t)q.y << 32));
        } else {
            if constexpr (SA) {
                lds_put<1>(lds, base[F::alpha] + u, q.x & 0xFF);
                lds_put<1>(lds, base[F::a1] + u, (q.x >> 8) & 0xFF);
            } else {
                lds_put<2, NAT>(lds, base[F::alpha] + 2 * u, q.x & 0xFFFF);
            }
            if constexpr (NAT && DXTLT_BC3_RECORD6) {
                lds_put_record6(lds, base[F::aidx] + 6 * u, q.x >> 16, q.y);
            } else {
                lds_put<2, NAT>(lds, base[F::aidx] + 6 * u + 0, q.x >> 16);
                lds_put<2, NAT>(lds, base[F::aidx] + 6 * u + 2, q.y & 0xFFFF);
                lds_put<2, NAT>(lds, base[F::aidx] + 6 * u + 4, q.y >> 16);
            }
        }
        if constexpr (SC) {
            lds_put<2, NAT>(lds, base[F::col] + 2 * u, c & 0xFFFF);
            lds_put<2, NAT>(lds, base[F::c1] + 2 * u, c >> 16);
        } else {
            lds_put<4, NAT>(lds, base[F::col] + 4 * u, c);
        }
        lds_put<4, NAT>(lds, base[F::idx] + 4 * u, q.w);
    }
}

template <int FMT, int VARIANT, bool SA, bool SC, bool NAT>
__device__ __forceinline__ u32x4 gather_shifted(uint8_t* lds, int u, const int (&base)[6])
{
    using F = FieldStreams<FMT, SA, SC>;
    u32x4 q;
    if constexpr (FMT == kBc4 || FMT == kBc5) {
        constexpr bool two = FMT == kBc4;
        uint32_t alo, ahi, blo, bhi;
        gather_shifted_bc4_block<SA, NAT, F::alpha, F::a1, F::aidx>(lds, two ? 2 * u : u, alo, ahi, base);
        if constexpr (two)
            gather_shifted_bc4_block<SA, NAT, F::alpha, F::a1, F::aidx>(lds, 2 * u + 1, blo, bhi, base);
        else
            gather_shifted_bc4_block<SA, NAT, F::galpha, F::ga1, F::gaidx>(lds, u, blo, bhi, base);
        q = u32x4{alo, ahi, blo, bhi};
    } else if constexpr (FMT == kBc1) {
        uint32_t ca, cb;
        uint64_t idx;
        if constexpr (NAT) {
            if constexpr (SC) {
                ca = (uint32_t)lds_get<2, true>(lds, base[F::col] + 4 * u) | ((uint32_t)lds_get<2, true>(lds, base[F::c1] + 4 * u) << 16);
                cb = (uint32_t)lds_get<2, true>(lds, base[F::col] + 4 * u + 2) |
                     ((uint32_t)lds_get<2, true>(lds, base[F::c1] + 4 * u + 2) << 16);
            } else {
                ca = (uint32_t)lds_get<4, true>(lds, base[F::col] + 8 * u);
                cb = (uint32_t)lds_get<4, true>(lds, base[F::col] + 8 * u + 4);
            }
            idx = lds_get<4, true>(lds, base[F::idx] + 8 * u) | (lds_get<4, true>(lds, base[F::idx] + 8 * u + 4) << 32);
        } else {
            if constexpr (SC) {
                const uint32_t c0 = (uint32_t)lds_get<4>(lds, base[F::col] + 4 * u);
                const uint32_t c1 = (uint32_t)lds_get<4>(lds, base[F::c1] + 4 * u);
                ca = (c0 & 0xFFFFu) | (c1 << 16);
                cb = (c0 >> 16) | (c1 & 0xFFFF0000u);
            } else {
                const uint64_t p = lds_get<8>(lds, base[F::col] + 8 * u);
                ca = (uint32_t)p;
                cb = (uint32_t)(p >> 32);
            }
            idx = lds_get<8>(lds, base[F::idx] + 8 * u);
        }
        q.x = recorrelate2<VARIANT>(ca);
        q.y = (uint32_t)idx;
        q.z = recorrelate2<VARIANT>(cb);
        q.w = (uint32_t)(idx >> 32);
    } else {
        if constexpr (FMT == kBc2) {
            const uint64_t a = lds_get<8, NAT>(lds, base[F::alpha] + 8 * u);
            q.x = (uint32_t)a;
            q.y = (uint32_t)(a >> 32);
        } else {
            uint32_t a01;
            if constexpr (SA)
                a01 = (uint32_t)lds_get<1>(lds, base[F::alpha] + u) | ((uint32_t)lds_get<1>(lds, base[F::a1] + u) << 8);
            else
                a01 = (uint32_t)lds_get<2, NAT>(lds, base[F::alpha] + 2 * u);
            if constexpr (NAT && DXTLT_BC3_RECORD6) {
                uint32_t i01, i2345;
                lds_get_record6(lds, base[F::aidx] + 6 * u, i01, i2345);
                q.x = a01 | (i01 << 16);
                q.y = i2345;
            } else {
                const uint32_t i01 = (uint32_t)lds_get<2, NAT>(lds, base[F::aidx] + 6 * u + 0);
                const uint32_t i23 = (uint32_t)lds_get<2, NAT>(lds, base[F::aidx] + 6 * u + 2);
                const uint32_t i45 = (uint32_t)lds_get<2, NAT>(lds, base[F::aidx] + 6 * u + 4);
                q.x = a01 | (i01 << 16);
                q.y = i23 | (i45 << 16);
            }
        }
        uint32_t c;
        if constexpr (SC)
            c = (uint32_t)lds_get<2, NAT>(lds, base[F::col] + 2 * u) | ((uint32_t)lds_get<2, NAT>(lds, base[F::c1] + 2 * u) << 16);
        else
            c = (uint32_t)lds_get<4, NAT>(lds, base[F::col] + 4 * u);
        q.z = recorrelate2<VARIANT>(c);
        q.w = (uint32_t)lds_get<4, NAT>(lds, base[F::idx] + 4 * u);
    }
    return q;
}

template <bool TO_GLOBAL>
__device__ __forceinline__ void copy_partial_segment(uint8_t* dst, const uint8_t* src, int lo, int hi)
{
    auto mv = [&](int p, int w) {
        if (w == 1) dst[p] = src[p];
        if (w == 2) *reinterpret_cast<uint16_t*>(dst + p) = *reinterpret_cast<const uint16_t*>(src + p);
        if (w == 4) *reinterpret_cast<uint32_t*>(dst + p) = *reinterpret_cast<const uint32_t*>(src + p);
        if (w == 8) *reinterpret_cast<u32x2*>(dst + p) = *reinterpret_cast<const u32x2*>(src + p);
    };
    if (hi == 16) {
        int p = lo;
        if (p & 1) { mv(p, 1); p += 1; }
        if (p & 2) { mv(p, 2); p += 2; }
        if (p & 4) { mv(p, 4); p += 4; }
        if (p & 8) { mv(p, 8); }
    } else {
        int p = 0;
        if (hi & 8) { mv(p, 8); p += 8; }
        if (hi & 4) { mv(p, 4); p += 4; }
        if (hi & 2) { mv(p, 2); p += 2; }
        if (hi & 1) { mv(p, 1); }
    }
}

__device__ __forceinline__ uint64_t uniform64(uint64_t v)
{
    return ((uint64_t)(uint32_t)__builtin_amdgcn_readfirstlane((int)(uint32_t)(v >> 32)) << 32) |
           (uint32_t)__builtin_amdgcn_readfirstlane((int)(uint32_t)v);
}

template <int FMT, bool SA, bool SC, int T>
__device__ __forceinline__ void slice_bases(uint64_t tile, const Shifts& sh, uint64_t (&gb)[6])
{
    constexpr Streams S = make_streams(FMT, SA, SC);
#pragma unroll
    for (int s = 0; s < 6; ++s)
        gb[s] = s < S.n ? uniform64(sh.gbase[s] + tile * (uint64_t)(S.width[s] * T)) : 0;
}

constexpr int shift_lds_bytes(int r, int threads = 256) { return r * threads * 16 + 16 * 6; }
constexpr int kShiftLdsBytes = shift_lds_bytes(1);

#ifndef DXTLT_BC1_SHIFT_THREADS
#define DXTLT_BC1_SHIFT_THREADS 256
#endif
__host__ __device__ constexpr int shift_tile_threads(int fmt) { return fmt == kBc1 ? DXTLT_BC1_SHIFT_THREADS : 256; }
__host__ __device__ constexpr int halo_tile_threads(int fmt, bool split_colour)
{
    return fmt == kBc1 && !split_colour ? 128 : shift_tile_threads(fmt);
}
#ifndef DXTLT_BATCH_BC1_NOSPLIT_FWD_THREADS
#define DXTLT_BATCH_BC1_NOSPLIT_FWD_THREADS 128
#endif
__host__ __device__ constexpr int batch_tile_threads(int fmt, bool split_colour, bool inverse)
{
    return !inverse && fmt == kBc1 && !split_colour ? DXTLT_BATCH_BC1_NOSPLIT_FWD_THREADS : shift_tile_threads(fmt);
}


#ifndef DXTLT_HALO_ALIGN
#define DXTLT_HALO_ALIGN 64
#endif
constexpr int kHaloAlign = DXTLT_HALO_ALIGN;
constexpr int kHaloBlocks = kHaloAlign;
constexpr int kHaloPad = kHaloAlign;
template <int FMT, int THREADS = 256>
constexpr int halo_lds_bytes() { return fmt_block(FMT) * (tile_blocks(FMT, THREADS) + kHaloBlocks) + kHaloPad * 6; }

__device__ __forceinline__ void copy_segment_bytes(uint8_t* dst, const uint8_t* src, int lo, int hi)
{
    int p = lo;
#pragma clang loop vectorize(disable) unroll(disable)
    while (p < hi) {
        const int left = hi - p;
        if ((p & 7) == 0 && left >= 8) {
            *reinterpret_cast<u32x2*>(dst + p) = *reinterpret_cast<const u32x2*>(src + p);
            p += 8;
        } else if ((p & 3) == 0 && left >= 4) {
            *reinterpret_cast<uint32_t*>(dst + p) = *reinterpret_cast<const uint32_t*>(src + p);
            p += 4;
        } else if ((p & 1) == 0 && left >= 2) {
            *reinterpret_cast<uint16_t*>(dst + p) = *reinterpret_cast<const uint16_t*>(src + p);
            p += 2;
        } else {
            dst[p] = src[p];
            p += 1;
        }
    }
}

template <int FMT, bool SA, bool SC, int W, bool EDGE = false, int THREADS = 256>
__device__ __forceinline__ void halo_copy_out_wave(uint8_t* __restrict__ soa, const uint8_t* lds, int t, const uint64_t (&gb)[6],
                                                   const Shifts& sh, const int (&vlo)[6], const int (&vhi)[6])
{
    constexpr Streams S = make_streams(FMT, SA, SC);
    constexpr int T = tile_blocks(FMT, THREADS);
    constexpr int H = kHaloBlocks;
    constexpr int wave_lo = W * 1024, wave_hi = wave_lo + 1024;
    const int o = t * 16;
    int la = 0, wo = 0, lo_s = 0, hi_s = 0;
    uint64_t g = 0;
    static_for<0, S.n>([&](auto si) {
        constexpr int s = decltype(si)::value;
        constexpr int lo = S.off[s] * T;
        constexpr int hi = lo + S.width[s] * T;
        if constexpr (lo < wave_hi && hi > wave_lo) {
            constexpr bool only = lo <= wave_lo && hi >= wave_hi;
            if (only || (o >= lo && o < hi)) {
                la = S.off[s] * (T + H) + kHaloPad * s + S.width[s] * H + (o - lo);
                g = gb[s] + (uint64_t)(o - lo);
                if constexpr (EDGE) {
                    wo = o - lo;
                    lo_s = vlo[s];
                    hi_s = vhi[s];
                }
            }
        }
    });
    if constexpr (EDGE) {
        const int lo = lo_s - wo > 0 ? lo_s - wo : 0;
        const int hi = hi_s - wo < 16 ? hi_s - wo : 16;
        if (hi <= lo)
            return;
        if (lo != 0 || hi != 16)
            copy_segment_bytes(soa + g, lds + la, lo, hi);
        else
            __builtin_nontemporal_store(lds_at<u32x4>(const_cast<uint8_t*>(lds), la), reinterpret_cast<u32x4*>(soa + g));
        return;
    }
    if (shifts_halo_write_through(sh))
        gstore16(soa + g, lds_at<u32x4>(const_cast<uint8_t*>(lds), la));
    else
        __builtin_nontemporal_store(lds_at<u32x4>(const_cast<uint8_t*>(lds), la), reinterpret_cast<u32x4*>(soa + g));
}

template <int FMT, int VARIANT, bool SA, bool SC, int NORM, bool NAT, int THREADS = 256>
__device__ __forceinline__ void fwd_halo_tile(const uint8_t* __restrict__ aos, uint8_t* __restrict__ soa,
                                              uint64_t , uint64_t , const Shifts& sh, uint64_t tile,
                                              uint8_t* lds)
{
    constexpr Streams S = make_streams(FMT, SA, SC);
    constexpr int T = tile_blocks(FMT, THREADS);
    constexpr int H = kHaloBlocks;
    constexpr int HV = H * fmt_block(FMT) / 16;
    const int t = threadIdx.x;
    int base[6];
#pragma unroll
    for (int s = 0; s < 6; ++s)
        base[s] = s < S.n ? S.off[s] * (T + H) + kHaloPad * s + sh.d[s] + S.width[s] * H : 0;

    const uint8_t* tile_aos = aos + tile * (THREADS * 16);
    WG_MARK(1);
    const u32x4 q = *reinterpret_cast<const u32x4*>(tile_aos + t * 16);
    const int hv = sh.halo_vecs;
    const bool has_halo = tile > 0 && t < hv && !shifts_skip_partial(sh);
    if (has_halo) {
        const u32x4 qh = *reinterpret_cast<const u32x4*>(tile_aos - hv * 16 + t * 16);
        scatter_shifted<FMT, VARIANT, SA, SC, NAT>(lds, t - hv, normalize_vector<FMT, NORM>(qh), base);
    }
    static_assert(HV <= THREADS, "the halo is loaded by the first lanes of the workgroup");
    WG_MARK_LOADS_DONE(2);
    scatter_shifted<FMT, VARIANT, SA, SC, NAT>(lds, t, normalize_vector<FMT, NORM>(q), base);
    __syncthreads();
    WG_MARK(3);

    uint64_t gb[6];
    slice_bases<FMT, SA, SC, T>(tile, sh, gb);
    const int none[6] = {0, 0, 0, 0, 0, 0};
    if constexpr (THREADS == 256) {
        switch (__builtin_amdgcn_readfirstlane(t >> 6)) {
        case 0: halo_copy_out_wave<FMT, SA, SC, 0>(soa, lds, t, gb, sh, none, none); break;
        case 1: halo_copy_out_wave<FMT, SA, SC, 1>(soa, lds, t, gb, sh, none, none); break;
        case 2: halo_copy_out_wave<FMT, SA, SC, 2>(soa, lds, t, gb, sh, none, none); break;
        default: halo_copy_out_wave<FMT, SA, SC, 3>(soa, lds, t, gb, sh, none, none); break;
        }
    } else {
        for_this_wave<THREADS / 64>(t, [&](auto wi) {
            halo_copy_out_wave<FMT, SA, SC, decltype(wi)::value, false, THREADS>(soa, lds, t, gb, sh, none, none);
        });
    }
    WG_MARK(4);
}

struct EdgeSlot {
    int s;
    int wo;
    int width;
    int d;
    int lds_base;
    uint64_t g;
};

template <int FMT, bool SA, bool SC, int T, int LA, int LB, int LC>
__device__ __forceinline__ EdgeSlot edge_slot_of_image_byte(int o, const Shifts& sh, const uint64_t (&gb)[6])
{
    constexpr Streams S = make_streams(FMT, SA, SC);
    EdgeSlot e{0, 0, 1, 0, 0, 0};
    static_for<0, S.n>([&](auto si) {
        constexpr int s = decltype(si)::value;
        constexpr int lo = S.off[s] * T, hi = lo + S.width[s] * T;
        if (o >= lo && o < hi) {
            e.s = s;
            e.wo = o - lo;
            e.width = S.width[s];
            e.d = sh.d[s];
            e.lds_base = S.off[s] * LA + LB * s + S.width[s] * LC;
            e.g = gb[s];
        }
    });
    return e;
}

template <int FMT, bool SA, bool SC, int T, int LA, int LB, int LC>
__device__ __forceinline__ EdgeSlot edge_slot_behind_window(int s_sel, int k, const Shifts& sh, const uint64_t (&gb)[6])
{
    constexpr Streams S = make_streams(FMT, SA, SC);
    EdgeSlot e{0, 0, 1, 0, 0, 0};
    static_for<0, S.n>([&](auto si) {
        constexpr int s = decltype(si)::value;
        if (s == s_sel) {
            e.s = s;
            e.wo = S.width[s] * T + 16 * k;
            e.width = S.width[s];
            e.d = sh.d[s];
            e.lds_base = S.off[s] * LA + LB * s + S.width[s] * LC;
            e.g = gb[s];
        }
    });
    return e;
}

template <int FMT, int VARIANT, bool SA, bool SC, int NORM, bool NAT, int THREADS = 256>
__device__ __forceinline__ void fwd_halo_edge_tile(const uint8_t* __restrict__ aos, uint8_t* __restrict__ soa, const Shifts& sh,
                                                   uint64_t tile, uint8_t* lds)
{
    constexpr Streams S = make_streams(FMT, SA, SC);
    constexpr int T = tile_blocks(FMT, THREADS);
    constexpr int H = kHaloBlocks;
    constexpr int PV = 16 / fmt_block(FMT);
    const int t = threadIdx.x;
    int base[6];
#pragma unroll
    for (int s = 0; s < 6; ++s)
        base[s] = s < S.n ? S.off[s] * (T + H) + kHaloPad * s + sh.d[s] + S.width[s] * H : 0;

    const uint64_t left = sh.range_blocks - tile * (uint64_t)T;
    const int own = left < (uint64_t)T ? (int)left : T;
    const uint8_t* tile_aos = aos + tile * (THREADS * 16);
    const int hv = sh.halo_vecs;
    const bool has_halo = tile > 0 && t < hv;
    const bool whole_vec = (t + 1) * PV <= own;
    const bool half_vec = PV == 2 && !whole_vec && t * PV < own;
    u32x4 q = {0u, 0u, 0u, 0u}, qh = {0u, 0u, 0u, 0u};
    if (whole_vec)
        q = *reinterpret_cast<const u32x4*>(tile_aos + t * 16);
    if (half_vec) {
        const u32x2 h = *reinterpret_cast<const u32x2*>(tile_aos + t * 16);
        q = u32x4{h.x, h.y, 0u, 0u};
    }
    if (has_halo)
        qh = *reinterpret_cast<const u32x4*>(tile_aos - hv * 16 + t * 16);
    if (has_halo)
        scatter_shifted<FMT, VARIANT, SA, SC, NAT>(lds, t - hv, normalize_vector<FMT, NORM>(qh), base);
    if (whole_vec || half_vec)
        scatter_shifted<FMT, VARIANT, SA, SC, NAT>(lds, t, normalize_vector<FMT, NORM>(q), base);
    __syncthreads();

    uint64_t gb[6];
    slice_bases<FMT, SA, SC, T>(tile, sh, gb);
    int vlo[6], vhi[6];
#pragma unroll
    for (int s = 0; s < 6; ++s) {
        const int d = s < S.n ? sh.d[s] : 0, w = s < S.n ? S.width[s] : 0;
        vlo[s] = tile == 0 ? d : 0;
        vhi[s] = own == T ? w * T : d + w * own;
    }
    if constexpr (THREADS == 256) {
        switch (__builtin_amdgcn_readfirstlane(t >> 6)) {
        case 0: halo_copy_out_wave<FMT, SA, SC, 0, true>(soa, lds, t, gb, sh, vlo, vhi); break;
        case 1: halo_copy_out_wave<FMT, SA, SC, 1, true>(soa, lds, t, gb, sh, vlo, vhi); break;
        case 2: halo_copy_out_wave<FMT, SA, SC, 2, true>(soa, lds, t, gb, sh, vlo, vhi); break;
        default: halo_copy_out_wave<FMT, SA, SC, 3, true>(soa, lds, t, gb, sh, vlo, vhi); break;
        }
    } else {
        for_this_wave<THREADS / 64>(t, [&](auto wi) {
            halo_copy_out_wave<FMT, SA, SC, decltype(wi)::value, true, THREADS>(soa, lds, t, gb, sh, vlo, vhi);
        });
    }
    constexpr int XS = kHaloAlign / 16;
    if (t < XS * S.n) {
        const EdgeSlot e = edge_slot_behind_window<FMT, SA, SC, T, T + H, kHaloPad, H>(t / XS, t % XS, sh, gb);
        int hi_s = 0;
#pragma unroll
        for (int s = 0; s < 6; ++s)
            hi_s = s == e.s ? vhi[s] : hi_s;
        const int hi = hi_s - e.wo < 16 ? hi_s - e.wo : 16;
        if (hi > 0) {
            uint8_t* la = lds + e.lds_base + e.wo;
            uint8_t* g = soa + e.g + (uint64_t)(int64_t)e.wo;
            if (hi != 16)
                copy_segment_bytes(g, la, 0, hi);
            else
                __builtin_nontemporal_store(*reinterpret_cast<u32x4*>(la), reinterpret_cast<u32x4*>(g));
        }
    }
}

template <int FMT, int VARIANT, bool SA, bool SC, int NORM, bool NAT, int THREADS = 256>
__global__ void __launch_bounds__(THREADS)
fwd_tiled_halo(const uint8_t* __restrict__ aos_arg, uint8_t* __restrict__ soa_arg, uint64_t total_blocks, uint64_t first_block,
               Shifts sh_arg)
{
    __shared__ __attribute__((aligned(16))) uint8_t lds[halo_lds_bytes<FMT, THREADS>()];
    WG_MARK(0);
    const uint32_t wg = blockIdx.x;
    const Shifts sh = shifts_fetched_at_once(sh_arg);
    const uint8_t* __restrict__ aos = fetched_now(aos_arg);
    uint8_t* __restrict__ soa = fetched_now(soa_arg);
    const bool whole = wg < sh.full_tiles;
    const uint64_t tile = !whole ? (uint64_t)sh.full_tiles : shifts_xcd_contiguous(sh, false) ? xcd_contiguous_tile(wg, sh.full_tiles) : (uint64_t)wg;
    const bool edge = !whole || tile == 0;
    if (edge)
        fwd_halo_edge_tile<FMT, VARIANT, SA, SC, NORM, NAT, THREADS>(aos, soa, sh, tile, lds);
    else
        fwd_halo_tile<FMT, VARIANT, SA, SC, NORM, NAT, THREADS>(aos, soa, total_blocks, first_block, sh, tile, lds);
}

template <int FMT, bool SA, bool SC, int W, int THREADS = 256>
__device__ __forceinline__ void inv_shift_load_wave(const uint8_t* __restrict__ soa, uint8_t* lds, int t,
                                                    const uint64_t (&gb)[6], const Shifts& sh, uint64_t total_bytes)
{
    constexpr Streams S = make_streams(FMT, SA, SC);
    constexpr int T = tile_blocks(FMT, THREADS);
    constexpr int wave_lo = W * 1024, wave_hi = wave_lo + 1024;
    const int o = t * 16;
    int la = 0, k = 0, shift = 0;
    uint64_t g = 0;
    static_for<0, S.n>([&](auto si) {
        constexpr int s = decltype(si)::value;
        constexpr int lo = S.off[s] * T;
        constexpr int hi = lo + S.width[s] * T;
        if constexpr (lo < wave_hi && hi > wave_lo) {
            constexpr bool only = lo <= wave_lo && hi >= wave_hi;
            if (only || (o >= lo && o < hi)) {
                la = lo + 16 * s + (o - lo);
                g = gb[s] + (uint64_t)(o - lo);
                k = (o - lo) >> 4;
                shift = sh.d[s];
            }
        }
    });
    const bool main_inside = g + 16 <= total_bytes;
    int la_t = 0, shift_t = 0;
    uint64_t g_t = 0;
    bool has_tail = false, tail_inside = false;
    if constexpr (W == 0) {
#pragma unroll
        for (int ss = 0; ss < S.n; ++ss) {
            if (ss == t) {
                const int bytes = S.width[ss] * T;
                la_t = S.off[ss] * T + 16 * ss + bytes;
                shift_t = sh.d[ss];
                g_t = gb[ss] + bytes;
            }
        }
        has_tail = t < S.n && shift_t > 0;
        tail_inside = g_t + 16 <= total_bytes;
    }
    u32x4 v_main = {0, 0, 0, 0}, v_tail = {0, 0, 0, 0};
    int tail_flags = (has_tail ? 1 : 0) | (tail_inside ? 2 : 0);
    asm volatile("" : "+v"(v_main), "+v"(v_tail), "+v"(g_t), "+v"(tail_flags));
    has_tail = (tail_flags & 1) != 0;
    tail_inside = (tail_flags & 2) != 0;
    if (main_inside)
        v_main = gload16(soa + g);
    if constexpr (W == 0) {
        if (has_tail && tail_inside)
            v_tail = gload16(soa + g_t);
        if (has_tail) {
            if (tail_inside)
                lds_at<u32x4>(lds, la_t) = v_tail;
            else
                copy_partial_segment<false>(lds + la_t, soa + g_t, 0, shift_t);
        }
    }
    if (main_inside)
        lds_at<u32x4>(lds, la) = v_main;
    else
        copy_partial_segment<false>(lds + la, soa + g, (k == 0) ? shift : 0, (k == 0) ? 16 : shift);
}

template <int FMT, int VARIANT, bool SA, bool SC, int THREADS = 256, typename SINK = AosSink>
__device__ __forceinline__ void inv_shift_tile(const uint8_t* __restrict__ soa, uint8_t* __restrict__ aos,
                                               uint64_t total_blocks, uint64_t , const Shifts& sh, uint64_t tile,
                                               uint8_t* lds, const SINK& sink = SINK{})
{
    constexpr Streams S = make_streams(FMT, SA, SC);
    constexpr int T = tile_blocks(FMT, THREADS);
    const int t = threadIdx.x;
    int base[6];
#pragma unroll
    for (int s = 0; s < 6; ++s)
        base[s] = s < S.n ? S.off[s] * T + 16 * s + sh.d[s] : 0;

    const uint64_t total_bytes = total_blocks * (uint64_t)fmt_block(FMT);
    uint64_t gb[6];
    slice_bases<FMT, SA, SC, T>(tile, sh, gb);
    if constexpr (THREADS == 256) {
        switch (__builtin_amdgcn_readfirstlane(t >> 6)) {
        case 0: inv_shift_load_wave<FMT, SA, SC, 0>(soa, lds, t, gb, sh, total_bytes); break;
        case 1: inv_shift_load_wave<FMT, SA, SC, 1>(soa, lds, t, gb, sh, total_bytes); break;
        case 2: inv_shift_load_wave<FMT, SA, SC, 2>(soa, lds, t, gb, sh, total_bytes); break;
        default: inv_shift_load_wave<FMT, SA, SC, 3>(soa, lds, t, gb, sh, total_bytes); break;
        }
    } else {
        for_this_wave<THREADS / 64>(t, [&](auto wi) {
            inv_shift_load_wave<FMT, SA, SC, decltype(wi)::value, THREADS>(soa, lds, t, gb, sh, total_bytes);
        });
    }
    __syncthreads();
    const u32x4 q = sh.natural ? gather_shifted<FMT, VARIANT, SA, SC, true>(lds, t, base)
                               : gather_shifted<FMT, VARIANT, SA, SC, false>(lds, t, base);
    sink.template store<FMT, THREADS>(aos, tile, t, q);
}

template <int FMT, int VARIANT, bool SA, bool SC, int THREADS = 256, typename SINK = AosSink>
__device__ __forceinline__ void inv_shift_edge_tile(const uint8_t* __restrict__ soa, uint8_t* __restrict__ aos,
                                                    uint64_t total_blocks, const Shifts& sh, uint64_t tile, uint8_t* lds,
                                                    const SINK& sink = SINK{})
{
    constexpr Streams S = make_streams(FMT, SA, SC);
    constexpr int T = tile_blocks(FMT, THREADS);
    constexpr int PV = 16 / fmt_block(FMT);
    const int t = threadIdx.x;
    int base[6];
#pragma unroll
    for (int s = 0; s < 6; ++s)
        base[s] = s < S.n ? S.off[s] * T + 16 * s + sh.d[s] : 0;
    const uint64_t left = sh.range_blocks - tile * (uint64_t)T;
    const int own = left < (uint64_t)T ? (int)left : T;
    const uint64_t total_bytes = total_blocks * (uint64_t)fmt_block(FMT);
    uint64_t gb[6];
    slice_bases<FMT, SA, SC, T>(tile, sh, gb);
    auto plan = [&](const EdgeSlot& e, int& lo, int& hi, bool& whole) {
        const int vhi = e.d + e.width * own;
        lo = e.d - e.wo > 0 ? e.d - e.wo : 0;
        hi = vhi - e.wo < 16 ? vhi - e.wo : 16;
        const uint64_t g = e.g + (uint64_t)(int64_t)e.wo;
        whole = total_bytes >= 16 && g <= total_bytes - 16;
    };
    const EdgeSlot em = edge_slot_of_image_byte<FMT, SA, SC, T, T, 16, 0>(t * 16, sh, gb);
    const EdgeSlot ex = edge_slot_behind_window<FMT, SA, SC, T, T, 16, 0>(t, 0, sh, gb);
    int mlo, mhi, xlo = 0, xhi = 0;
    bool mwhole, xwhole = false;
    plan(em, mlo, mhi, mwhole);
    if (t < S.n)
        plan(ex, xlo, xhi, xwhole);
    const uint8_t* gm = soa + em.g + (uint64_t)(int64_t)em.wo;
    const uint8_t* gx = soa + ex.g + (uint64_t)(int64_t)ex.wo;
    u32x4 vm = {0u, 0u, 0u, 0u}, vx = {0u, 0u, 0u, 0u};
    if (mhi > mlo && mwhole)
        vm = *reinterpret_cast<const u32x4*>(gm);
    if (xhi > xlo && xwhole)
        vx = *reinterpret_cast<const u32x4*>(gx);
    if (mhi > mlo) {
        if (mwhole)
            *reinterpret_cast<u32x4*>(lds + em.lds_base + em.wo) = vm;
        else
            copy_segment_bytes(lds + em.lds_base + em.wo, gm, mlo, mhi);
    }
    if (xhi > xlo) {
        if (xwhole)
            *reinterpret_cast<u32x4*>(lds + ex.lds_base + ex.wo) = vx;
        else
            copy_segment_bytes(lds + ex.lds_base + ex.wo, gx, xlo, xhi);
    }
    __builtin_amdgcn_s_waitcnt(0x0F70);
    __syncthreads();
    if (t * PV < own) {
        const u32x4 q = sh.natural ? gather_shifted<FMT, VARIANT, SA, SC, true>(lds, t, base)
                                   : gather_shifted<FMT, VARIANT, SA, SC, false>(lds, t, base);
        sink.template store_edge<FMT, THREADS>(aos, tile, t, q, own);
    }
}

template <int FMT, int VARIANT, bool SA, bool SC, int THREADS = 256>
__global__ void __launch_bounds__(THREADS)
inv_tiled_shift(const uint8_t* __restrict__ soa_arg, uint8_t* __restrict__ aos_arg, uint64_t total_blocks, uint64_t first_block,
                Shifts sh_arg)
{
    __shared__ __attribute__((aligned(16))) uint8_t lds[shift_lds_bytes(1, THREADS)];
    const uint32_t wg = blockIdx.x;
    const Shifts sh = shifts_fetched_at_once(sh_arg);
    const uint8_t* __restrict__ soa = fetched_now(soa_arg);
    uint8_t* __restrict__ aos = fetched_now(aos_arg);
    asm("" : "+s"(total_blocks));
    const bool whole = wg < sh.full_tiles;
    const uint64_t tile = !whole ? (uint64_t)sh.full_tiles : shifts_xcd_contiguous(sh, true) ? xcd_contiguous_tile(wg, sh.full_tiles) : (uint64_t)wg;
    const bool edge = !whole;
    if (edge)
        inv_shift_edge_tile<FMT, VARIANT, SA, SC, THREADS>(soa, aos, total_blocks, sh, tile, lds);
    else
        inv_shift_tile<FMT, VARIANT, SA, SC, THREADS>(soa, aos, total_blocks, first_block, sh, tile, lds);
}

template <int W>
__device__ __forceinline__ void store_bytes(uint8_t* p, uint64_t v, bool natural)
{
    if (natural) {
        if constexpr (W == 1) *p = (uint8_t)v;
        if constexpr (W == 2) *reinterpret_cast<uint16_t*>(p) = (uint16_t)v;
        if constexpr (W == 4) *reinterpret_cast<uint32_t*>(p) = (uint32_t)v;
        if constexpr (W == 8) *reinterpret_cast<uint64_t*>(p) = v;
    } else {
#pragma unroll
        for (int i = 0; i < W; ++i)
            p[i] = (uint8_t)(v >> (8 * i));
    }
}

template <int W>
__device__ __forceinline__ uint64_t load_bytes(const uint8_t* p, bool natural)
{
    if (natural) {
        if constexpr (W == 1) return *p;
        if constexpr (W == 2) return *reinterpret_cast<const uint16_t*>(p);
        if constexpr (W == 4) return *reinterpret_cast<const uint32_t*>(p);
        if constexpr (W == 8) return *reinterpret_cast<const uint64_t*>(p);
    }
    uint64_t v = 0;
#pragma unroll
    for (int i = 0; i < W; ++i)
        v |= (uint64_t)p[i] << (8 * i);
    return v;
}

__device__ __forceinline__ bool aligned_to(const void* p, int a) { return (reinterpret_cast<uintptr_t>(p) & (a - 1)) == 0; }


}

#ifdef DXTLT_EXPERIMENTS
#include "bcn_experiments.h"
#endif
```

### dxt-lossless-transform_amd/csrc/bcn_launch.h

```cpp
#pragma once
#include <hip/hip_runtime_api.h>
#include <stddef.h>
#include <stdint.h>

#include <cstdlib>

namespace dxtlt {

inline const char* experiment_env(const char* name)
{
#ifdef DXTLT_EXPERIMENTS
    return std::getenv(name);
#else
    (void)name;
    return nullptr;
#endif
}

enum Format : int { kBc1 = 1, kBc2 = 2, kBc3 = 3, kBc4 = 4, kBc5 = 5 };

struct Settings {
    int variant;
    bool split_alpha;
    bool split_colour;
    int normalize = 0;
};

struct Range {
    uint64_t total_blocks;
    uint64_t first_block;
    uint64_t num_blocks;
};

struct LaunchTuning {
    int tile_threads;
    int force_generic;
    int xcd_remap;
};

int launch_force_mask();

struct DebugPlannedLaunch {
    int32_t kind;
    int32_t threads;
    uint32_t workgroups;
    uint32_t full_tiles;
    uint64_t range_blocks;
    uint64_t aos_offset;
    uint8_t shift[6];
    uint8_t halo_vecs;
    uint8_t natural;
    uint64_t gbase[6];
};
int debug_plan_transform(Format fmt, bool inverse, const Settings& s, uint64_t src_address, uint64_t dst_address, const Range& r,
                         const LaunchTuning* tuning, DebugPlannedLaunch* out, int cap);

hipError_t launch_transform(Format fmt, bool inverse, const Settings& s, const void* src, void* dst,
                            const Range& r, hipStream_t stream, const LaunchTuning* tuning = nullptr);

hipError_t launch_fill_splitmix64(void* dst, size_t len_bytes, uint64_t seed, uint64_t first_qword,
                                  hipStream_t stream);

hipError_t launch_normalize_bc1_blocks(const void* in, void* out, uint64_t num_blocks, int mode, hipStream_t stream);
hipError_t launch_normalize_bc1_split(void* colours, void* indices, uint64_t num_blocks, int mode, hipStream_t stream);
hipError_t launch_normalize_bc1_all_modes(const void* in, void* const out[3], uint64_t num_blocks, uint32_t* d_any,
                                          hipStream_t stream);
hipError_t launch_bc1_any_normalizable(const void* in, uint64_t num_blocks, uint32_t* d_any, hipStream_t stream);

hipError_t launch_decode_blocks(int fmt, const void* in, void* out, uint64_t num_blocks, hipStream_t stream);
hipError_t launch_count_pixel_differences(int fmt, const void* a, const void* b, uint64_t num_blocks, uint64_t* d_count,
                                          hipStream_t stream);

hipError_t launch_color565_ycocg(bool inverse, const void* in, void* out, uint64_t num_items, int variant, hipStream_t stream);
hipError_t launch_color565_recorrelate_split(const void* src0, const void* src1, void* dst, uint64_t num_items, int variant,
                                             hipStream_t stream);
hipError_t launch_split_565_color_endpoints(const void* in, void* out, uint64_t len_bytes, hipStream_t stream);

hipError_t launch_normalize_bc23_blocks(int fmt, const void* in, void* out, uint64_t num_blocks, int alpha_mode, int color_mode,
                                        hipStream_t stream);
hipError_t launch_normalize_bc23_all_modes(int fmt, const void* in, void* const* outs, uint64_t num_blocks, hipStream_t stream);
hipError_t launch_normalize_bc2_split(void* colours, void* indices, uint64_t num_blocks, int color_mode, hipStream_t stream);
hipError_t launch_normalize_bc3_split(void* alpha_endpoints, void* alpha_indices, void* color_endpoints, void* color_indices,
                                      uint64_t num_blocks, int alpha_mode, int color_mode, hipStream_t stream);

struct BatchEntry {
    const uint8_t* src;
    uint8_t* dst;
    uint64_t blocks;
    uint32_t first_wg;
    uint32_t end_wg;
    uint32_t full_tiles;
    uint8_t form;
    uint8_t halo_vecs;
    uint8_t natural;
    uint8_t reserved;
    uint8_t shift[6];
    uint8_t reserved2[2];
    uint64_t gbase[6];
};
static_assert(sizeof(BatchEntry) == 96, "BatchEntry layout is shared between host and device");

constexpr uint32_t kBatchIndexWgs = 64, kBatchBaseWgs = 4096;
inline size_t batch_index_base_count(uint32_t total_wgs) { return ((size_t)total_wgs + kBatchBaseWgs - 1) / kBatchBaseWgs; }
inline size_t batch_index_delta_count(uint32_t total_wgs) { return ((size_t)total_wgs + kBatchIndexWgs - 1) / kBatchIndexWgs; }
inline size_t batch_index_bytes(uint32_t total_wgs)
{
    return (batch_index_base_count(total_wgs) * 4 + 2 * batch_index_delta_count(total_wgs) + 15) & ~(size_t)15;
}

uint32_t plan_batch_entry(Format fmt, bool inverse, const Settings& s, BatchEntry& e);

hipError_t launch_table_upload(const void* host_mapped, void* dev, size_t bytes, hipStream_t stream);

hipError_t launch_batch(Format fmt, bool inverse, const Settings& s, const BatchEntry* d_entries, const uint8_t* d_index,
                        uint32_t n_entries, uint32_t total_wgs, uint32_t uniform_wgs, bool wide_index, hipStream_t stream,
                        const BatchEntry* strided_first = nullptr, int64_t src_stride = 0, int64_t dst_stride = 0);

bool build_batch_index(const BatchEntry* entries, size_t n_entries, uint32_t total_wgs, uint8_t* index);

hipError_t launch_tiled_array(Format fmt, bool inverse, const Settings& s, const void* first_src, void* first_dst,
                              uint64_t blocks, uint32_t n_buffers, int64_t src_stride, int64_t dst_stride, hipStream_t stream);

inline int block_bytes(Format f) { return f == kBc1 || f == kBc4 ? 8 : 16; }

constexpr bool format_has_alpha_split(int fmt) { return fmt == kBc3 || fmt == kBc4 || fmt == kBc5; }
constexpr bool format_has_colour(int fmt) { return fmt == kBc1 || fmt == kBc2 || fmt == kBc3; }
inline Settings effective_settings(Format f, const Settings& s)
{
    Settings e = s;
    e.split_alpha = format_has_alpha_split(f) && s.split_alpha;
    if (!format_has_colour(f)) {
        e.variant = 0;
        e.split_colour = false;
    }
    return e;
}

struct Streams {
    int n;
    int width[6];
    int off[6];
};

constexpr Streams make_streams(int fmt, bool split_alpha, bool split_colour)
{
    Streams s{};
    int n = 0, off = 0;
    if (fmt == kBc4 || fmt == kBc5) {
        for (int h = 0; h < (fmt == kBc5 ? 2 : 1); ++h) {
            if (split_alpha) {
                s.width[n] = 1; s.off[n] = off; off += 1; ++n;
                s.width[n] = 1; s.off[n] = off; off += 1; ++n;
            } else {
                s.width[n] = 2; s.off[n] = off; off += 2; ++n;
            }
            s.width[n] = 6; s.off[n] = off; off += 6; ++n;
        }
        s.n = n;
        return s;
    }
    if (fmt == kBc3) {
        if (split_alpha) {
            s.width[n] = 1; s.off[n] = off; off += 1; ++n;
            s.width[n] = 1; s.off[n] = off; off += 1; ++n;
        } else {
            s.width[n] = 2; s.off[n] = off; off += 2; ++n;
        }
        s.width[n] = 6; s.off[n] = off; off += 6; ++n;
    }
    if (fmt == kBc2) {
        s.width[n] = 8; s.off[n] = off; off += 8; ++n;
    }
    if (split_colour) {
        s.width[n] = 2; s.off[n] = off; off += 2; ++n;
        s.width[n] = 2; s.off[n] = off; off += 2; ++n;
    } else {
        s.width[n] = 4; s.off[n] = off; off += 4; ++n;
    }
    s.width[n] = 4; s.off[n] = off; off += 4; ++n;
    s.n = n;
    return s;
}

}
```

Measured before the change: 3159.

## Precompute batch entry rotation and whole-tile count to trim kernel prologue

```diff
diff --git a/dxt-lossless-transform_amd/csrc/batch_api.cpp b/dxt-lossless-transform_amd/csrc/batch_api.cpp
--- a/dxt-lossless-transform_amd/csrc/batch_api.cpp
+++ b/dxt-lossless-transform_amd/csrc/batch_api.cpp
@@ -124,7 +124,7 @@
         e.dst = static_cast<uint8_t*>(it.d_output);
         e.blocks = it.len / item_block_bytes(it.format);
         e.first_wg = g.wgs;
-        const uint32_t wgs = dxtlt::plan_batch_entry((dxtlt::Format)it.format, it.inverse != 0, group_settings(gi), e);
+        const uint32_t wgs = dxtlt::plan_batch_entry((dxtlt::Format)it.format, it.inverse != 0, group_settings(gi), e, (uint32_t)g.entries.size());
         if (wgs == 0xFFFFFFFFu) {
             singles.push_back(i);
             continue;
@@ -241,7 +241,7 @@
             const int64_t dst_stride = n >= 2 ? (int64_t)(g.entries[1].dst - g.entries[0].dst) : 0;
             for (size_t i = 1; i < n && strided; ++i) {
                 const BatchEntry &a = g.entries[0], &b = g.entries[i];
-                strided = b.blocks == a.blocks && b.full_tiles == a.full_tiles && b.form == a.form && b.halo_vecs == a.halo_vecs &&
+                strided = b.blocks == a.blocks && b.full_tiles == a.full_tiles && b.form_whole == a.form_whole && b.halo_vecs == a.halo_vecs &&
                           std::memcmp(b.shift, a.shift, sizeof a.shift) == 0 && std::memcmp(b.gbase, a.gbase, sizeof a.gbase) == 0 &&
                           b.src == a.src + (int64_t)i * src_stride && b.dst == a.dst + (int64_t)i * dst_stride;
             }
@@ -306,7 +306,7 @@
         e.dst = reinterpret_cast<uint8_t*>(static_cast<uintptr_t>(dst_addresses[i]));
         e.blocks = blocks[i];
         e.first_wg = total;
-        const uint32_t wgs = dxtlt::plan_batch_entry((dxtlt::Format)format, inverse != 0, s, e);
+        const uint32_t wgs = dxtlt::plan_batch_entry((dxtlt::Format)format, inverse != 0, s, e, (uint32_t)entries.size());
         if (wgs == 0xFFFFFFFFu || (uint64_t)total + wgs > 0xFFFFFFull)
             return 0xFFFFFFFFu;
         if (wgs == 0)
@@ -316,7 +316,7 @@
         o.first_wg = e.first_wg;
         o.end_wg = e.end_wg;
         o.full_tiles = e.full_tiles;
-        o.form = e.form;
+        o.form = (uint8_t)(e.form_whole & 1u);
         o.halo_vecs = e.halo_vecs;
         std::memcpy(o.shift, e.shift, sizeof o.shift);
         std::memcpy(o.gbase, e.gbase, sizeof o.gbase);
diff --git a/dxt-lossless-transform_amd/csrc/batch_kernels.hip b/dxt-lossless-transform_amd/csrc/batch_kernels.hip
--- a/dxt-lossless-transform_amd/csrc/batch_kernels.hip
+++ b/dxt-lossless-transform_amd/csrc/batch_kernels.hip
@@ -13,7 +13,7 @@
     uint8_t* dst;
     uint64_t blocks;
     uint32_t first_wg, end_wg, full_tiles;
-    uint32_t flags;
+    uint32_t form_whole;
     uint32_t shifts[2];
     uint64_t gbase[6];
 };
@@ -29,7 +29,7 @@
     v.first_wg = w[6];
     v.end_wg = w[7];
     v.full_tiles = w[8];
-    v.flags = w[9];
+    v.form_whole = w[9];
     v.shifts[0] = w[10];
     v.shifts[1] = w[11];
 #pragma unroll
@@ -47,16 +47,15 @@
     asm("" : "+s"(s), "+s"(d), "+s"(v.blocks));
     v.src = (const uint8_t*)(global_cptr)s;
     v.dst = (uint8_t*)(global_ptr)d;
-    asm("" : "+s"(v.first_wg), "+s"(v.end_wg), "+s"(v.full_tiles), "+s"(v.flags), "+s"(v.shifts[0]), "+s"(v.shifts[1]));
+    asm("" : "+s"(v.first_wg), "+s"(v.end_wg), "+s"(v.full_tiles), "+s"(v.form_whole), "+s"(v.shifts[0]), "+s"(v.shifts[1]));
 #pragma unroll
     for (int i = 0; i < 6; ++i)
         asm("" : "+s"(v.gbase[i]));
 }
-static_assert(offsetof(BatchEntry, first_wg) == 24 && offsetof(BatchEntry, end_wg) == 28 && offsetof(BatchEntry, full_tiles) == 32 && offsetof(BatchEntry, form) == 36 &&
-                  offsetof(BatchEntry, shift) == 40 && offsetof(BatchEntry, gbase) == 48,
+static_assert(offsetof(BatchEntry, first_wg) == 24 && offsetof(BatchEntry, end_wg) == 28 && offsetof(BatchEntry, full_tiles) == 32 && offsetof(BatchEntry, form_whole) == 36 &&
+                  offsetof(BatchEntry, shift) == 40 && offsetof(BatchEntry, halo_vecs) == 46 && offsetof(BatchEntry, rotation) == 47 && offsetof(BatchEntry, gbase) == 48,
               "load_batch_entry reads BatchEntry by dword offsets");
 
-constexpr uint32_t kBatchAligned = 1;
 
 struct StridedBatch {
     BatchEntry first;
@@ -95,8 +94,8 @@
 
 template <int FMT, int VARIANT, bool SA, bool SC, bool INVERSE, int THREADS = batch_tile_threads(FMT, SC, INVERSE)>
 __global__ void __launch_bounds__(THREADS)
-batch_kernel(const BatchEntry* __restrict__ entries_arg, const uint8_t* __restrict__ index_arg, uint32_t n_base, uint32_t uniform_wgs,
-             uint32_t magic, StridedBatch strided)
+batch_kernel(const BatchEntry* __restrict__ entries_arg, const uint8_t* __restrict__ index_arg, const uint8_t* __restrict__ delta_arg,
+             BatchIndexForm index_form, uint32_t uniform_wgs, uint32_t magic, StridedBatch strided)
 {
     constexpr int kLds = INVERSE ? shift_lds_bytes(1, THREADS) : halo_lds_bytes<FMT, THREADS>();
     __shared__ __attribute__((aligned(16))) uint8_t lds[kLds];
@@ -104,12 +103,16 @@
     WG_TIMING_BEGIN
     BatchView en;
     uint32_t e;
+    uint32_t rotation;
     uint64_t entries_at = reinterpret_cast<uintptr_t>(entries_arg), index_at = reinterpret_cast<uintptr_t>(index_arg);
+    uint64_t delta_at = reinterpret_cast<uintptr_t>(delta_arg);
 #ifndef DXTLT_WG_TIMING
-    asm("" : "+s"(entries_at), "+s"(index_at), "+s"(n_base), "+s"(uniform_wgs), "+s"(magic));
+    asm("" : "+s"(entries_at), "+s"(index_at), "+s"(delta_at), "+s"(index_form.dword_shift), "+s"(index_form.slot_mask),
+             "+s"(index_form.slot_shift), "+s"(index_form.value_mask), "+s"(uniform_wgs), "+s"(magic));
 #endif
     const BatchEntry* entries = (const BatchEntry*)(const __attribute__((address_space(1))) BatchEntry*)entries_at;
     const uint8_t* index = (const uint8_t*)(global_cptr)index_at;
+    const uint8_t* delta = (const uint8_t*)(global_cptr)delta_at;
     if (uniform_wgs != 0) {
         e = __umulhi(wg, magic);
         if ((e + 1) * uniform_wgs <= wg)
@@ -122,26 +125,52 @@
             en.first_wg = e * uniform_wgs;
             en.end_wg = en.first_wg + uniform_wgs;
             en.full_tiles = f.full_tiles;
-            en.flags = (uint32_t)f.form | ((uint32_t)f.halo_vecs << 8) | ((uint32_t)f.natural << 16);
+            en.form_whole = f.form_whole;
             en.shifts[0] = (uint32_t)f.shift[0] | ((uint32_t)f.shift[1] << 8) | ((uint32_t)f.shift[2] << 16) | ((uint32_t)f.shift[3] << 24);
-            en.shifts[1] = (uint32_t)f.shift[4] | ((uint32_t)f.shift[5] << 8);
+            en.shifts[1] = (uint32_t)f.shift[4] | ((uint32_t)f.shift[5] << 8) | ((uint32_t)f.halo_vecs << 16);
 #pragma unroll
             for (int i = 0; i < 6; ++i)
                 en.gbase[i] = f.gbase[i];
+            rotation = batch_entry_rotation(en.first_wg, en.end_wg, e);
         } else {
             en = load_batch_entry(entries + e);
+            rotation = en.shifts[1] >> 24;
         }
     } else {
-        e = batch_entry_of_workgroup(entries, index, n_base, magic, wg, en);
+        e = batch_entry_of_workgroup(entries, index, delta, index_form, magic, wg, en);
+        rotation = en.shifts[1] >> 24;
     }
     const uint32_t n_wgs = en.end_wg - en.first_wg;
-    uint32_t local = wg - en.first_wg;
-    if (n_wgs >= 8) {
-        local += (en.first_wg + n_wgs - 1u - e) & 7u;
-        local = local >= n_wgs ? local - n_wgs : local;
-    }
-    const bool aligned = (en.flags & 0xFF) == kBatchAligned;
-    if (aligned && local < en.full_tiles) {
+    uint32_t local = wg - en.first_wg + rotation;
+    local = local < local - n_wgs ? local : local - n_wgs;
+    constexpr Streams S = make_streams(FMT, SA, SC);
+    constexpr uint32_t kFirstWhole = INVERSE ? 0 : 1;
+    Shifts sh;
+#pragma unroll
+    for (int i = 0; i < 6; ++i) {
+        sh.d[i] = i < S.n ? (int)((en.shifts[i >> 2] >> (8 * (i & 3))) & 127u) : 0;
+        sh.gbase[i] = en.gbase[i];
+    }
+#ifdef DXTLT_EXPERIMENTS
+    sh.xcd_remap = 0;
+    sh.line_policy = INVERSE ? 1 : 3;
+    sh.skip_partial = 0;
+#endif
+    sh.natural = 1;
+    sh.halo_vecs = (int)(en.shifts[1] >> 16) & 0xFF;
+    sh.full_tiles = en.full_tiles;
+    sh.range_blocks = en.blocks;
+    if (local - kFirstWhole < en.form_whole >> 8) {
+        if constexpr (INVERSE) {
+            const uint64_t tile = xcd_contiguous_tile(local, en.full_tiles);
+            inv_shift_tile<FMT, VARIANT, SA, SC, THREADS>(en.src, en.dst, en.blocks, 0, sh, tile, lds);
+        } else {
+            fwd_halo_tile<FMT, VARIANT, SA, SC, kNormNone, true, THREADS>(en.src, en.dst, en.blocks, 0, sh, local, lds);
+        }
+        WG_TIMING_END(2);
+        return;
+    }
+    if ((en.form_whole & 1u) != 0 && local < en.full_tiles) {
         if constexpr (INVERSE)
             inv_aligned_tile<FMT, VARIANT, SA, SC, THREADS>(en.src, en.dst, en.blocks, 0, local, lds);
         else
@@ -149,42 +178,16 @@
         WG_TIMING_END(1);
         return;
     }
-    Shifts sh;
-#pragma unroll
-    for (int i = 0; i < 6; ++i) {
-        sh.d[i] = (int)((en.shifts[i >> 2] >> (8 * (i & 3))) & 127u);
-        sh.gbase[i] = en.gbase[i];
-    }
-#ifdef DXTLT_EXPERIMENTS
-    sh.xcd_remap = 0;
-    sh.line_policy = INVERSE ? 1 : 3;
-    sh.skip_partial = 0;
-#endif
-    sh.natural = 1;
-    sh.halo_vecs = (int)(en.flags >> 8) & 0xFF;
-    sh.full_tiles = en.full_tiles;
-    sh.range_blocks = en.blocks;
     if constexpr (INVERSE) {
-        if (local < en.full_tiles) {
-            const uint64_t tile = xcd_contiguous_tile(local, en.full_tiles);
-            inv_shift_tile<FMT, VARIANT, SA, SC, THREADS>(en.src, en.dst, en.blocks, 0, sh, tile, lds);
-            WG_TIMING_END(2);
-            return;
-        }
         inv_shift_edge_tile<FMT, VARIANT, SA, SC, THREADS>(en.src, en.dst, en.blocks, sh, en.full_tiles, lds);
         WG_TIMING_END(4);
     } else {
-        if (local != 0 && local < en.full_tiles) {
-            fwd_halo_tile<FMT, VARIANT, SA, SC, kNormNone, true, THREADS>(en.src, en.dst, en.blocks, 0, sh, local, lds);
-            WG_TIMING_END(2);
-            return;
-        }
         fwd_halo_edge_tile<FMT, VARIANT, SA, SC, kNormNone, true, THREADS>(en.src, en.dst, sh, local, lds);
         WG_TIMING_END(local == 0 ? 3 : 4);
     }
 }
 
-uint32_t plan_batch_entry(Format fmt, bool inverse, const Settings& s, BatchEntry& e)
+uint32_t plan_batch_entry(Format fmt, bool inverse, const Settings& s, BatchEntry& e, uint32_t index_in_launch)
 {
     if (e.blocks == 0)
         return 0;
@@ -205,10 +208,6 @@
     }
     if (!shifts_are_natural(S, d))
         return 0xFFFFFFFFu;
-    e.form = on_lines ? 1 : 0;
-    e.natural = 1;
-    e.reserved = 0;
-    e.reserved2[0] = e.reserved2[1] = 0;
     const int per_vec = 16 / fmt_block(fmt);
     e.halo_vecs = inverse ? 0 : (uint8_t)((halo_blocks + per_vec - 1) / per_vec);
     for (int i = 0; i < 6; ++i) {
@@ -216,9 +215,13 @@
         e.gbase[i] = i < S.n ? (uint64_t)S.off[i] * e.blocks - (uint64_t)d[i] : 0;
     }
     e.full_tiles = (uint32_t)tiles;
+    const uint32_t first_whole = inverse ? 0u : 1u;
+    const uint32_t whole = !on_lines && tiles > first_whole ? (uint32_t)tiles - first_whole : 0u;
+    e.form_whole = (on_lines ? 1u : 0u) | (whole << 8);
     const bool edge = rest != 0 || (!inverse && stream_tails);
     const uint32_t wgs = (uint32_t)tiles + (edge ? 1u : 0u);
     e.end_wg = e.first_wg + wgs;
+    e.rotation = (uint8_t)batch_entry_rotation(e.first_wg, e.end_wg, index_in_launch);
     return wgs;
 }
 
@@ -254,7 +257,7 @@
 
 namespace {
 
-using BatchFn = void (*)(const BatchEntry*, const uint8_t*, uint32_t, uint32_t, uint32_t, StridedBatch);
+using BatchFn = void (*)(const BatchEntry*, const uint8_t*, const uint8_t*, BatchIndexForm, uint32_t, uint32_t, StridedBatch);
 
 template <int FMT, int VARIANT, bool SA, bool SC>
 BatchFn batch_fn(bool inverse) { return inverse ? batch_kernel<FMT, VARIANT, SA, SC, true> : batch_kernel<FMT, VARIANT, SA, SC, false>; }
@@ -300,7 +303,7 @@
         return hipErrorInvalidValue;
     const uint32_t magic = uniform_wgs > 1 ? (uint32_t)((1ull << 32) / uniform_wgs) : uniform_wgs == 1 ? 0xFFFFFFFFu : n_entries;
     static const bool no_array = experiment_env("DXTLT_BATCH_NO_ARRAY") != nullptr;
-    if (strided_first != nullptr && uniform_wgs != 0 && !no_array && strided_first->form == 1) {
+    if (strided_first != nullptr && uniform_wgs != 0 && !no_array && (strided_first->form_whole & 1u) != 0) {
         const hipError_t e = launch_tiled_array(fmt, inverse, s, strided_first->src, strided_first->dst, strided_first->blocks, n_entries,
                                                 src_stride, dst_stride, stream);
         if (e != hipErrorNotSupported)
@@ -325,7 +328,7 @@
     default: return hipErrorInvalidValue;
     }
     hipLaunchKernelGGL(k, dim3(total_wgs), dim3(batch_tile_threads(fmt, sc, inverse)), 0, stream, d_entries, d_index,
-                       (uint32_t)batch_index_base_count(total_wgs) | (wide_index ? 0x80000000u : 0u), uniform_wgs, magic, strided);
+                       d_index + batch_index_base_count(total_wgs) * 4, batch_index_form(wide_index ? 1u : 0u), uniform_wgs, magic, strided);
     return hipGetLastError();
 }
 
diff --git a/dxt-lossless-transform_amd/csrc/batch_lookup.h b/dxt-lossless-transform_amd/csrc/batch_lookup.h
--- a/dxt-lossless-transform_amd/csrc/batch_lookup.h
+++ b/dxt-lossless-transform_amd/csrc/batch_lookup.h
@@ -4,17 +4,27 @@
 
 namespace dxtlt {
 
+struct BatchIndexForm {
+    uint32_t dword_shift;
+    uint32_t slot_mask;
+    uint32_t slot_shift;
+    uint32_t value_mask;
+};
+__host__ __device__ inline BatchIndexForm batch_index_form(uint32_t wide)
+{
+    return BatchIndexForm{8u - wide, 3u >> wide, 3u + wide, 0xFFu | (wide * 0xFF00u)};
+}
+
 template <typename ENTRY, typename VIEW>
-__device__ __forceinline__ uint32_t batch_entry_of_workgroup(const ENTRY* entries, const uint8_t* index, uint32_t n_base,
-                                                             uint32_t n_entries, uint32_t wg, VIEW& en)
+__device__ __forceinline__ uint32_t batch_entry_of_workgroup(const ENTRY* entries, const uint8_t* base_index, const uint8_t* delta,
+                                                             const BatchIndexForm& form, uint32_t n_entries, uint32_t wg, VIEW& en)
 {
     static_assert(offsetof(ENTRY, end_wg) == 28, "the bisection reads end_wg as dword 7 of an entry");
-    const uint32_t* base = reinterpret_cast<const uint32_t*>(index);
-    const uint32_t wide = n_base >> 31;
-    const uint8_t* delta = index + (n_base & 0x7FFFFFFFu) * 4;
+    const uint32_t* base = reinterpret_cast<const uint32_t*>(base_index);
     uint32_t e = base[wg >> 12];
-    const uint32_t dword = reinterpret_cast<const uint32_t*>(delta)[wg >> (8u - wide)];
-    e += (dword >> (((wg >> 6) & (3u >> wide)) << (3u + wide))) & (0xFFu | (wide * 0xFF00u));
+    __builtin_amdgcn_sched_barrier(0);
+    const uint32_t dword = reinterpret_cast<const uint32_t*>(delta)[wg >> form.dword_shift];
+    e += (dword >> (((wg >> 6) & form.slot_mask) << form.slot_shift)) & form.value_mask;
     en = load_batch_entry(entries + e);
     pin_batch_view(en);
     if (en.end_wg <= wg) {
@@ -32,6 +42,13 @@
     return e;
 }
 
+template <typename ENTRY, typename VIEW>
+__device__ __forceinline__ uint32_t batch_entry_of_workgroup(const ENTRY* entries, const uint8_t* index, uint32_t n_base,
+                                                             uint32_t n_entries, uint32_t wg, VIEW& en)
+{
+    return batch_entry_of_workgroup(entries, index, index + (n_base & 0x7FFFFFFFu) * 4, batch_index_form(n_base >> 31), n_entries, wg, en);
+}
+
 __device__ __forceinline__ uint32_t batch_rotated_tile(uint32_t first_wg, uint32_t end_wg, uint32_t e, uint32_t wg)
 {
     const uint32_t n_wgs = end_wg - first_wg;
diff --git a/dxt-lossless-transform_amd/csrc/bcn_device.h b/dxt-lossless-transform_amd/csrc/bcn_device.h
--- a/dxt-lossless-transform_amd/csrc/bcn_device.h
+++ b/dxt-lossless-transform_amd/csrc/bcn_device.h
@@ -358,7 +358,7 @@
 __device__ __forceinline__ uint64_t xcd_contiguous_tile(uint32_t orig, uint32_t nwg)
 {
     const uint32_t q = nwg >> 3, r = nwg & 7, xcd = orig & 7;
-    const uint32_t start = xcd < r ? xcd * (q + 1) : r * (q + 1) + (xcd - r) * q;
+    const uint32_t start = xcd * q + (xcd < r ? xcd : r);
     return start + (orig >> 3);
 }
 
@@ -882,6 +882,13 @@
         gb[s] = s < S.n ? uniform64(sh.gbase[s] + tile * (uint64_t)(S.width[s] * T)) : 0;
 }
 
+template <int FMT, bool SA, bool SC, int T, int s>
+__device__ __forceinline__ uint64_t slice_base(uint64_t tile, const Shifts& sh)
+{
+    constexpr Streams S = make_streams(FMT, SA, SC);
+    return uniform64(sh.gbase[s] + (uint64_t)(uint32_t)tile * (uint32_t)(S.width[s] * T));
+}
+
 constexpr int shift_lds_bytes(int r, int threads = 256) { return r * threads * 16 + 16 * 6; }
 constexpr int kShiftLdsBytes = shift_lds_bytes(1);
 
@@ -902,6 +909,9 @@
 }
 
 
+#ifndef DXTLT_HALO_NT_LOADS
+#define DXTLT_HALO_NT_LOADS 0
+#endif
 #ifndef DXTLT_HALO_ALIGN
 #define DXTLT_HALO_ALIGN 64
 #endif
@@ -935,7 +945,7 @@
 
 template <int FMT, bool SA, bool SC, int W, bool EDGE = false, int THREADS = 256>
 __device__ __forceinline__ void halo_copy_out_wave(uint8_t* __restrict__ soa, const uint8_t* lds, int t, const uint64_t (&gb)[6],
-                                                   const Shifts& sh, const int (&vlo)[6], const int (&vhi)[6])
+                                                   const Shifts& sh, const int (&vlo)[6], const int (&vhi)[6], uint64_t tile = 0)
 {
     constexpr Streams S = make_streams(FMT, SA, SC);
     constexpr int T = tile_blocks(FMT, THREADS);
@@ -950,9 +960,10 @@
         constexpr int hi = lo + S.width[s] * T;
         if constexpr (lo < wave_hi && hi > wave_lo) {
             constexpr bool only = lo <= wave_lo && hi >= wave_hi;
+            const uint64_t gbs = EDGE ? gb[s] : slice_base<FMT, SA, SC, T, s>(tile, sh);
             if (only || (o >= lo && o < hi)) {
                 la = S.off[s] * (T + H) + kHaloPad * s + S.width[s] * H + (o - lo);
-                g = gb[s] + (uint64_t)(o - lo);
+                g = gbs + (uint64_t)(o - lo);
                 if constexpr (EDGE) {
                     wo = o - lo;
                     lo_s = vlo[s];
@@ -995,7 +1006,15 @@
 
     const uint8_t* tile_aos = aos + tile * (THREADS * 16);
     WG_MARK(1);
+#if DXTLT_HALO_NT_LOADS
+    u32x4 q;
+    if (__builtin_amdgcn_readfirstlane(t >> 6) == THREADS / 64 - 1)
+        q = *reinterpret_cast<const u32x4*>(tile_aos + t * 16);
+    else
+        q = gload16(tile_aos + t * 16);
+#else
     const u32x4 q = *reinterpret_cast<const u32x4*>(tile_aos + t * 16);
+#endif
     const int hv = sh.halo_vecs;
     const bool has_halo = tile > 0 && t < hv && !shifts_skip_partial(sh);
     if (has_halo) {
@@ -1008,19 +1027,18 @@
     __syncthreads();
     WG_MARK(3);
 
-    uint64_t gb[6];
-    slice_bases<FMT, SA, SC, T>(tile, sh, gb);
+    const uint64_t no_gb[6] = {0, 0, 0, 0, 0, 0};
     const int none[6] = {0, 0, 0, 0, 0, 0};
     if constexpr (THREADS == 256) {
         switch (__builtin_amdgcn_readfirstlane(t >> 6)) {
-        case 0: halo_copy_out_wave<FMT, SA, SC, 0>(soa, lds, t, gb, sh, none, none); break;
-        case 1: halo_copy_out_wave<FMT, SA, SC, 1>(soa, lds, t, gb, sh, none, none); break;
-        case 2: halo_copy_out_wave<FMT, SA, SC, 2>(soa, lds, t, gb, sh, none, none); break;
-        default: halo_copy_out_wave<FMT, SA, SC, 3>(soa, lds, t, gb, sh, none, none); break;
+        case 0: halo_copy_out_wave<FMT, SA, SC, 0>(soa, lds, t, no_gb, sh, none, none, tile); break;
+        case 1: halo_copy_out_wave<FMT, SA, SC, 1>(soa, lds, t, no_gb, sh, none, none, tile); break;
+        case 2: halo_copy_out_wave<FMT, SA, SC, 2>(soa, lds, t, no_gb, sh, none, none, tile); break;
+        default: halo_copy_out_wave<FMT, SA, SC, 3>(soa, lds, t, no_gb, sh, none, none, tile); break;
         }
     } else {
         for_this_wave<THREADS / 64>(t, [&](auto wi) {
-            halo_copy_out_wave<FMT, SA, SC, decltype(wi)::value, false, THREADS>(soa, lds, t, gb, sh, none, none);
+            halo_copy_out_wave<FMT, SA, SC, decltype(wi)::value, false, THREADS>(soa, lds, t, no_gb, sh, none, none, tile);
         });
     }
     WG_MARK(4);
@@ -1161,9 +1179,14 @@
     const Shifts sh = shifts_fetched_at_once(sh_arg);
     const uint8_t* __restrict__ aos = fetched_now(aos_arg);
     uint8_t* __restrict__ soa = fetched_now(soa_arg);
+#ifdef DXTLT_EXPERIMENTS
     const bool whole = wg < sh.full_tiles;
     const uint64_t tile = !whole ? (uint64_t)sh.full_tiles : shifts_xcd_contiguous(sh, false) ? xcd_contiguous_tile(wg, sh.full_tiles) : (uint64_t)wg;
     const bool edge = !whole || tile == 0;
+#else
+    const uint64_t tile = wg;
+    const bool edge = wg - 1u >= sh.full_tiles - 1u;
+#endif
     if (edge)
         fwd_halo_edge_tile<FMT, VARIANT, SA, SC, NORM, NAT, THREADS>(aos, soa, sh, tile, lds);
     else
@@ -1172,7 +1195,7 @@
 
 template <int FMT, bool SA, bool SC, int W, int THREADS = 256>
 __device__ __forceinline__ void inv_shift_load_wave(const uint8_t* __restrict__ soa, uint8_t* lds, int t,
-                                                    const uint64_t (&gb)[6], const Shifts& sh, uint64_t total_bytes)
+                                                    uint64_t tile, const Shifts& sh, uint64_t total_bytes)
 {
     constexpr Streams S = make_streams(FMT, SA, SC);
     constexpr int T = tile_blocks(FMT, THREADS);
@@ -1186,9 +1209,10 @@
         constexpr int hi = lo + S.width[s] * T;
         if constexpr (lo < wave_hi && hi > wave_lo) {
             constexpr bool only = lo <= wave_lo && hi >= wave_hi;
+            const uint64_t gbs = slice_base<FMT, SA, SC, T, s>(tile, sh);
             if (only || (o >= lo && o < hi)) {
                 la = lo + 16 * s + (o - lo);
-                g = gb[s] + (uint64_t)(o - lo);
+                g = gbs + (uint64_t)(o - lo);
                 k = (o - lo) >> 4;
                 shift = sh.d[s];
             }
@@ -1199,15 +1223,16 @@
     uint64_t g_t = 0;
     bool has_tail = false, tail_inside = false;
     if constexpr (W == 0) {
-#pragma unroll
-        for (int ss = 0; ss < S.n; ++ss) {
+        static_for<0, S.n>([&](auto ssi) {
+            constexpr int ss = decltype(ssi)::value;
+            const uint64_t gbs = slice_base<FMT, SA, SC, T, ss>(tile, sh);
             if (ss == t) {
                 const int bytes = S.width[ss] * T;
                 la_t = S.off[ss] * T + 16 * ss + bytes;
                 shift_t = sh.d[ss];
-                g_t = gb[ss] + bytes;
+                g_t = gbs + bytes;
             }
-        }
+        });
         has_tail = t < S.n && shift_t > 0;
         tail_inside = g_t + 16 <= total_bytes;
     }
@@ -1248,18 +1273,16 @@
         base[s] = s < S.n ? S.off[s] * T + 16 * s + sh.d[s] : 0;
 
     const uint64_t total_bytes = total_blocks * (uint64_t)fmt_block(FMT);
-    uint64_t gb[6];
-    slice_bases<FMT, SA, SC, T>(tile, sh, gb);
     if constexpr (THREADS == 256) {
         switch (__builtin_amdgcn_readfirstlane(t >> 6)) {
-        case 0: inv_shift_load_wave<FMT, SA, SC, 0>(soa, lds, t, gb, sh, total_bytes); break;
-        case 1: inv_shift_load_wave<FMT, SA, SC, 1>(soa, lds, t, gb, sh, total_bytes); break;
-        case 2: inv_shift_load_wave<FMT, SA, SC, 2>(soa, lds, t, gb, sh, total_bytes); break;
-        default: inv_shift_load_wave<FMT, SA, SC, 3>(soa, lds, t, gb, sh, total_bytes); break;
+        case 0: inv_shift_load_wave<FMT, SA, SC, 0>(soa, lds, t, tile, sh, total_bytes); break;
+        case 1: inv_shift_load_wave<FMT, SA, SC, 1>(soa, lds, t, tile, sh, total_bytes); break;
+        case 2: inv_shift_load_wave<FMT, SA, SC, 2>(soa, lds, t, tile, sh, total_bytes); break;
+        default: inv_shift_load_wave<FMT, SA, SC, 3>(soa, lds, t, tile, sh, total_bytes); break;
         }
     } else {
         for_this_wave<THREADS / 64>(t, [&](auto wi) {
-            inv_shift_load_wave<FMT, SA, SC, decltype(wi)::value, THREADS>(soa, lds, t, gb, sh, total_bytes);
+            inv_shift_load_wave<FMT, SA, SC, decltype(wi)::value, THREADS>(soa, lds, t, tile, sh, total_bytes);
         });
     }
     __syncthreads();
diff --git a/dxt-lossless-transform_amd/csrc/bcn_launch.h b/dxt-lossless-transform_amd/csrc/bcn_launch.h
--- a/dxt-lossless-transform_amd/csrc/bcn_launch.h
+++ b/dxt-lossless-transform_amd/csrc/bcn_launch.h
@@ -90,14 +90,16 @@
     uint32_t first_wg;
     uint32_t end_wg;
     uint32_t full_tiles;
-    uint8_t form;
+    uint32_t form_whole;
+    uint8_t shift[6];
     uint8_t halo_vecs;
-    uint8_t natural;
-    uint8_t reserved;
-    uint8_t shift[6];
-    uint8_t reserved2[2];
+    uint8_t rotation;
     uint64_t gbase[6];
 };
+__host__ __device__ inline uint32_t batch_entry_rotation(uint32_t first_wg, uint32_t end_wg, uint32_t index_in_launch)
+{
+    return end_wg - first_wg >= 8 ? (end_wg - 1u - index_in_launch) & 7u : 0u;
+}
 static_assert(sizeof(BatchEntry) == 96, "BatchEntry layout is shared between host and device");
 
 constexpr uint32_t kBatchIndexWgs = 64, kBatchBaseWgs = 4096;
@@ -108,7 +110,7 @@
     return (batch_index_base_count(total_wgs) * 4 + 2 * batch_index_delta_count(total_wgs) + 15) & ~(size_t)15;
 }
 
-uint32_t plan_batch_entry(Format fmt, bool inverse, const Settings& s, BatchEntry& e);
+uint32_t plan_batch_entry(Format fmt, bool inverse, const Settings& s, BatchEntry& e, uint32_t index_in_launch);
 
 hipError_t launch_table_upload(const void* host_mapped, void* dev, size_t bytes, hipStream_t stream);
 
```

New measurement: 3157. About the same (-0.1%).
